# facebookresearch/nonrigid_nerf

Measured on NVIDIA H100. Metric: rays/sec (64c+128f samples, 8x256 MLP), example_sequence training step, higher is better.
Workload: dtype f16 (tensor-core operands; f32 accumulate)

## Files before the change

include/nrnerf_b200.h:

```cpp
#ifndef NRNERF_B200_H
#define NRNERF_B200_H

#include <stddef.h>
#include <stdint.h>

#ifdef __cplusplus
extern "C" {
#endif

#define NRN_ABI_VERSION 3

#define NRN_OK 0
#define NRN_E_INVALID (-1)
#define NRN_E_CUDA (-2)
#define NRN_E_DEVICE (-3)

int nrn_abi_version(void);
const char* nrn_last_error(void);

int nrn_device_error(int* code_out);

size_t nrn_packed_nerf_bytes(void);
size_t nrn_packed_bender_bytes(void);
int nrn_pack_nerf(const float* const* w, const float* const* b, int input_ch, int out_ch, void* packed,
                  void* stream);
int nrn_pack_bender(const float* const* net_w , const float* const* net_b ,
                    const float* const* rig_w , const float* const* rig_b , int latent_size,
                    void* packed, void* stream);

int nrn_get_rays(const float* c2w, const float* intrinsics, int height, int width, float* rays_o, float* rays_d, void* stream);
int nrn_pack_rays(const float* rays_o, const float* rays_d, float near, float far, int n_rays, float* rays, void* stream);
int nrn_ray_batch(const int64_t* pix, int n, const float* poses, const float* intrinsics, const int32_t* image_to_view,
                  const float* images, int height, int width, float* rays_o, float* rays_d, float* target, void* stream);
int nrn_median_visibility_index(const float* weights, int n_rays, int n_samples, int64_t* index, void* stream);

int nrn_sample_coarse(const float* rays, const float* t_rand, int n_rays, int n_samples, int lindisp,
                      float* z_vals, void* stream);

typedef struct NrnFieldArgs {
  const float* rays;
  const float* z_vals;
  const float* points;
  int64_t points_stride;
  const float* latents;
  int64_t latent_stride;
  int32_t n_rays;
  int32_t n_samples;
  const void* nerf_packed;
  const void* bender_packed;
  int32_t out_ch;
  int32_t use_cutoff;  float rigidity_cutoff;
  int32_t use_scaling; float scaling;
  int32_t use_removal; float removal_threshold;
  float* raw;
  float* initial_input_pts;
  float* input_pts;
  float* unmasked_offsets;
  float* masked_offsets;
  float* rigidity_mask;
  void* stash;
  void* stream;
  void* relu_mask;
} NrnFieldArgs;
int nrn_field_forward(const NrnFieldArgs* args);

typedef struct NrnCompositeArgs {
  const float* raw;
  const float* z_vals;
  const float* rays_d;
  int32_t rays_d_stride;
  const float* noise;
  int32_t n_rays, n_samples, channels, white_bkgd;
  float* rgb_map;
  float* disp_map;
  float* acc_map;
  float* depth_map;
  float* weights;
  float* alpha;
  int32_t n_importance;
  const float* u;
  float* z_vals_out;
  float* z_std;
  void* stream;
} NrnCompositeArgs;
int nrn_composite(const NrnCompositeArgs* args);

int nrn_sample_pdf(const float* bins, const float* weights, const float* u, int n, int nbins, int n_samples,
                   float* samples, void* stream);

typedef struct NrnCompositeBwdArgs {
  const float* raw; const float* z_vals; const float* rays_d; int32_t rays_d_stride; const float* noise;
  int32_t n_rays, n_samples, channels, white_bkgd;
  const float* d_rgb_map;
  const float* d_acc_map;
  float* d_raw;
  void* stream;
} NrnCompositeBwdArgs;
int nrn_composite_backward(const NrnCompositeBwdArgs* args);

size_t nrn_stash_bytes(int n_rays, int n_samples);
size_t nrn_grad_stash_bytes(int n_rays, int n_samples);
size_t nrn_relu_mask_bytes(int n_rays, int n_samples);
size_t nrn_wgrad_scratch_bytes(void);
int nrn_nerf_grad_floats(int out_ch);
int nrn_bender_grad_floats(void);
typedef struct NrnFieldBwdArgs {
  int32_t n_rays, n_samples, out_ch;
  const float* d_raw;
  const void* stash;
  void* grad_stash;
  float* wgrad_scratch;
  const void* nerf_packed;
  const void* bender_packed;
  const float* unmasked_offsets;
  const float* rigidity_mask;
  const float* d_unmasked_offsets;
  const float* d_rigidity_mask;
  int32_t use_cutoff;  float rigidity_cutoff;
  int32_t use_scaling; float scaling;
  float* nerf_grad;
  float* bender_grad;
  float* d_latents;
  void* stream;
  float* nerf_grad_head;
  int32_t accumulate_nerf, accumulate_bender;
  const void* relu_mask;
} NrnFieldBwdArgs;
int nrn_field_backward(const NrnFieldBwdArgs* args);

size_t nrn_div_stash_bytes(int n_rays, int n_samples);
size_t nrn_div_grad_stash_bytes(int n_rays, int n_samples);
typedef struct NrnDivArgs {
  int32_t n_rays, n_samples;
  const void* stash;
  const float* e;
  const float* unmasked_offsets;
  const float* rigidity_mask;
  const float* weights;
  int32_t weights_are_opacity_alpha;
  const float* const* net_w;
  const float* const* rig_w;
  void* tangent_stash;
  float* d; float* alpha; float* beta; float* tau_c;
  float* loss;
  const float* G;
  const float* g_ray;
  float* G_workspace;
  void* adjoint_stash;
  float* wgrad_scratch;
  float* d_unmasked_offsets;
  float* d_rigidity_mask;
  float* bender_grad;
  void* stream;
  int32_t accumulate_bender;
} NrnDivArgs;
int nrn_divergence_forward(const NrnDivArgs* args);
int nrn_divergence_backward(const NrnDivArgs* args);

typedef struct NrnRayLossArgs {
  int32_t n_rays, n_samples;
  const float* rgb;
  const float* rgb0;
  const float* target;
  const float* weights;
  const float* unmasked_offsets;
  const float* rigidity_mask;
  float lam_offsets;
  float lam_rigidity;
  float* loss;
  float* u_rgb; float* u_rgb0;
  float* u_unmasked_offsets;
  float* u_rigidity_mask;
  void* stream;
  const float* sched_step;
  float sched_n_iters;
  const float* divergence;
  float lam_divergence;
  float* u_divergence;
} NrnRayLossArgs;
int nrn_ray_loss(const NrnRayLossArgs* args);
int nrn_scale_rows(const float* g, const float* unit, float* out, int64_t n, int per_row, void* stream);
typedef struct NrnRayLossBwdArgs {
  int32_t n_rays, n_samples;
  const float* g;
  const float* u_rgb; const float* u_rgb0; const float* u_unmasked_offsets; const float* u_rigidity_mask; const float* u_divergence;
  float* d_rgb; float* d_rgb0; float* d_unmasked_offsets; float* d_rigidity_mask; float* d_divergence;
  void* stream;
} NrnRayLossBwdArgs;
int nrn_ray_loss_backward(const NrnRayLossBwdArgs* args);

typedef struct NrnAdamArgs {
  void* params;
  void* exp_avg;
  void* exp_avg_sq;
  const void* grad_ptrs;
  const void* blocks;
  int n_tensors, n_blocks;
  const void* lr;
  void* step;
  float beta1, beta2, eps;
  void* stream;
} NrnAdamArgs;
int nrn_adam_step(const NrnAdamArgs* args);

size_t nrn_peer_window_bytes(int64_t arena_floats, int64_t slot_floats);
int nrn_peer_alloc(size_t bytes, void** dev_ptr, void* ipc_handle_64bytes);
int nrn_peer_open(const void* ipc_handle_64bytes, void** dev_ptr);
int nrn_peer_close(void* dev_ptr);
int nrn_peer_free(void* dev_ptr);
typedef struct NrnPeerCtx {
  void* window[8];
  int32_t world, rank;
  int64_t arena_floats, slot_floats;
  void* state;
  float* reduced;
} NrnPeerCtx;
int nrn_peer_reduce_adam(const NrnPeerCtx* ctx, const NrnAdamArgs* adam);
int nrn_peer_gather_rows(const NrnPeerCtx* ctx, const float* local, int n_per_rank, float* out, void* stream);

int nrn_timing_enable(int on);
int nrn_timing_read(double* ms_sum, int* counts, int n_kinds);

#ifdef __cplusplus
}
#endif
#endif
```

nonrigid_nerf_b200/_lib.py:

```python
from __future__ import annotations

import ctypes as C
import os
import threading

_HERE = os.path.dirname(os.path.abspath(__file__))
LIB_PATH = os.path.join(_HERE, "libnrnerf_b200.so")
ABI_VERSION = 3

_f32p = C.POINTER(C.c_float)
_vp = C.c_void_p


class NrnFieldArgs(C.Structure):
    _fields_ = [
        ("rays", _vp), ("z_vals", _vp), ("points", _vp), ("points_stride", C.c_int64),
        ("latents", _vp), ("latent_stride", C.c_int64),
        ("n_rays", C.c_int32), ("n_samples", C.c_int32),
        ("nerf_packed", _vp), ("bender_packed", _vp),
        ("out_ch", C.c_int32),
        ("use_cutoff", C.c_int32), ("rigidity_cutoff", C.c_float),
        ("use_scaling", C.c_int32), ("scaling", C.c_float),
        ("use_removal", C.c_int32), ("removal_threshold", C.c_float),
        ("raw", _vp), ("initial_input_pts", _vp), ("input_pts", _vp), ("unmasked_offsets", _vp),
        ("masked_offsets", _vp), ("rigidity_mask", _vp),
        ("stash", _vp),
        ("stream", _vp),
        ("relu_mask", _vp),
    ]


class NrnFieldBwdArgs(C.Structure):
    _fields_ = [
        ("n_rays", C.c_int32), ("n_samples", C.c_int32), ("out_ch", C.c_int32),
        ("d_raw", _vp), ("stash", _vp), ("grad_stash", _vp), ("wgrad_scratch", _vp),
        ("nerf_packed", _vp), ("bender_packed", _vp),
        ("unmasked_offsets", _vp), ("rigidity_mask", _vp), ("d_unmasked_offsets", _vp), ("d_rigidity_mask", _vp),
        ("use_cutoff", C.c_int32), ("rigidity_cutoff", C.c_float),
        ("use_scaling", C.c_int32), ("scaling", C.c_float),
        ("nerf_grad", _vp), ("bender_grad", _vp), ("d_latents", _vp),
        ("stream", _vp),
        ("nerf_grad_head", _vp), ("accumulate_nerf", C.c_int32), ("accumulate_bender", C.c_int32),
        ("relu_mask", _vp),
    ]


class NrnDivArgs(C.Structure):
    _fields_ = [
        ("n_rays", C.c_int32), ("n_samples", C.c_int32),
        ("stash", _vp), ("e", _vp), ("unmasked_offsets", _vp), ("rigidity_mask", _vp), ("weights", _vp),
        ("weights_are_opacity_alpha", C.c_int32),
        ("net_w", C.POINTER(_vp)), ("rig_w", C.POINTER(_vp)),
        ("tangent_stash", _vp), ("d", _vp), ("alpha", _vp), ("beta", _vp), ("tau_c", _vp), ("loss", _vp),
        ("G", _vp), ("g_ray", _vp), ("G_workspace", _vp), ("adjoint_stash", _vp), ("wgrad_scratch", _vp), ("d_unmasked_offsets", _vp),
        ("d_rigidity_mask", _vp), ("bender_grad", _vp),
        ("stream", _vp),
        ("accumulate_bender", C.c_int32),
    ]


class NrnRayLossArgs(C.Structure):
    _fields_ = [
        ("n_rays", C.c_int32), ("n_samples", C.c_int32),
        ("rgb", _vp), ("rgb0", _vp), ("target", _vp), ("weights", _vp), ("unmasked_offsets", _vp), ("rigidity_mask", _vp),
        ("lam_offsets", C.c_float), ("lam_rigidity", C.c_float),
        ("loss", _vp), ("u_rgb", _vp), ("u_rgb0", _vp), ("u_unmasked_offsets", _vp), ("u_rigidity_mask", _vp),
        ("stream", _vp),
        ("sched_step", _vp), ("sched_n_iters", C.c_float), ("divergence", _vp), ("lam_divergence", C.c_float), ("u_divergence", _vp),
    ]


class NrnRayLossBwdArgs(C.Structure):
    _fields_ = [
        ("n_rays", C.c_int32), ("n_samples", C.c_int32), ("g", _vp),
        ("u_rgb", _vp), ("u_rgb0", _vp), ("u_unmasked_offsets", _vp), ("u_rigidity_mask", _vp), ("u_divergence", _vp),
        ("d_rgb", _vp), ("d_rgb0", _vp), ("d_unmasked_offsets", _vp), ("d_rigidity_mask", _vp), ("d_divergence", _vp),
        ("stream", _vp),
    ]


class NrnAdamArgs(C.Structure):
    _fields_ = [
        ("params", _vp), ("exp_avg", _vp), ("exp_avg_sq", _vp), ("grad_ptrs", _vp), ("blocks", _vp), ("n_tensors", C.c_int32), ("n_blocks", C.c_int32),
        ("lr", _vp), ("step", _vp), ("beta1", C.c_float), ("beta2", C.c_float), ("eps", C.c_float), ("stream", _vp),
    ]


class NrnPeerCtx(C.Structure):
    _fields_ = [
        ("window", _vp * 8), ("world", C.c_int32), ("rank", C.c_int32), ("arena_floats", C.c_int64), ("slot_floats", C.c_int64),
        ("state", _vp), ("reduced", _vp),
    ]


class NrnCompositeArgs(C.Structure):
    _fields_ = [
        ("raw", _vp), ("z_vals", _vp), ("rays_d", _vp), ("rays_d_stride", C.c_int32), ("noise", _vp),
        ("n_rays", C.c_int32), ("n_samples", C.c_int32), ("channels", C.c_int32), ("white_bkgd", C.c_int32),
        ("rgb_map", _vp), ("disp_map", _vp), ("acc_map", _vp), ("depth_map", _vp), ("weights", _vp), ("alpha", _vp),
        ("n_importance", C.c_int32), ("u", _vp), ("z_vals_out", _vp), ("z_std", _vp),
        ("stream", _vp),
    ]


class NrnCompositeBwdArgs(C.Structure):
    _fields_ = [
        ("raw", _vp), ("z_vals", _vp), ("rays_d", _vp), ("rays_d_stride", C.c_int32), ("noise", _vp),
        ("n_rays", C.c_int32), ("n_samples", C.c_int32), ("channels", C.c_int32), ("white_bkgd", C.c_int32),
        ("d_rgb_map", _vp), ("d_acc_map", _vp), ("d_raw", _vp),
        ("stream", _vp),
    ]


SYMBOLS = {
    "nrn_abi_version": (C.c_int, []),
    "nrn_last_error": (C.c_char_p, []),
    "nrn_device_error": (C.c_int, [C.POINTER(C.c_int)]),
    "nrn_packed_nerf_bytes": (C.c_size_t, []),
    "nrn_packed_bender_bytes": (C.c_size_t, []),
    "nrn_pack_nerf": (C.c_int, [C.POINTER(_vp), C.POINTER(_vp), C.c_int, C.c_int, _vp, _vp]),
    "nrn_pack_bender": (C.c_int, [C.POINTER(_vp), C.POINTER(_vp), C.POINTER(_vp), C.POINTER(_vp), C.c_int, _vp, _vp]),
    "nrn_sample_coarse": (C.c_int, [_vp, _vp, C.c_int, C.c_int, C.c_int, _vp, _vp]),
    "nrn_get_rays": (C.c_int, [_vp, _vp, C.c_int, C.c_int, _vp, _vp, _vp]),
    "nrn_pack_rays": (C.c_int, [_vp, _vp, C.c_float, C.c_float, C.c_int, _vp, _vp]),
    "nrn_ray_batch": (C.c_int, [_vp, C.c_int, _vp, _vp, _vp, _vp, C.c_int, C.c_int, _vp, _vp, _vp, _vp]),
    "nrn_median_visibility_index": (C.c_int, [_vp, C.c_int, C.c_int, _vp, _vp]),
    "nrn_field_forward": (C.c_int, [C.POINTER(NrnFieldArgs)]),
    "nrn_composite": (C.c_int, [C.POINTER(NrnCompositeArgs)]),
    "nrn_sample_pdf": (C.c_int, [_vp, _vp, _vp, C.c_int, C.c_int, C.c_int, _vp, _vp]),
    "nrn_composite_backward": (C.c_int, [C.POINTER(NrnCompositeBwdArgs)]),
    "nrn_stash_bytes": (C.c_size_t, [C.c_int, C.c_int]),
    "nrn_grad_stash_bytes": (C.c_size_t, [C.c_int, C.c_int]),
    "nrn_relu_mask_bytes": (C.c_size_t, [C.c_int, C.c_int]),
    "nrn_wgrad_scratch_bytes": (C.c_size_t, []),
    "nrn_nerf_grad_floats": (C.c_int, [C.c_int]),
    "nrn_bender_grad_floats": (C.c_int, []),
    "nrn_field_backward": (C.c_int, [C.POINTER(NrnFieldBwdArgs)]),
    "nrn_div_stash_bytes": (C.c_size_t, [C.c_int, C.c_int]),
    "nrn_div_grad_stash_bytes": (C.c_size_t, [C.c_int, C.c_int]),
    "nrn_divergence_forward": (C.c_int, [C.POINTER(NrnDivArgs)]),
    "nrn_divergence_backward": (C.c_int, [C.POINTER(NrnDivArgs)]),
    "nrn_ray_loss": (C.c_int, [C.POINTER(NrnRayLossArgs)]),
    "nrn_scale_rows": (C.c_int, [_vp, _vp, _vp, C.c_int64, C.c_int, _vp]),
    "nrn_ray_loss_backward": (C.c_int, [C.POINTER(NrnRayLossBwdArgs)]),
    "nrn_adam_step": (C.c_int, [C.POINTER(NrnAdamArgs)]),
    "nrn_peer_window_bytes": (C.c_size_t, [C.c_int64, C.c_int64]),
    "nrn_peer_alloc": (C.c_int, [C.c_size_t, C.POINTER(_vp), C.c_char_p]),
    "nrn_peer_open": (C.c_int, [C.c_char_p, C.POINTER(_vp)]),
    "nrn_peer_close": (C.c_int, [_vp]),
    "nrn_peer_free": (C.c_int, [_vp]),
    "nrn_peer_reduce_adam": (C.c_int, [C.POINTER(NrnPeerCtx), C.POINTER(NrnAdamArgs)]),
    "nrn_peer_gather_rows": (C.c_int, [C.POINTER(NrnPeerCtx), _vp, C.c_int, _vp, _vp]),
    "nrn_timing_enable": (C.c_int, [C.c_int]),
    "nrn_timing_read": (C.c_int, [C.POINTER(C.c_double), C.POINTER(C.c_int), C.c_int]),
}

KERNEL_KINDS = ("field_fwd", "field_dgrad", "wgrad", "composite", "composite_bwd", "divergence")


def timing_enable(on: bool) -> None:
    check(load().nrn_timing_enable(1 if on else 0), "timing_enable")


def timing_read():
    n = len(KERNEL_KINDS)
    ms = (C.c_double * n)()
    cnt = (C.c_int * n)()
    check(load().nrn_timing_read(ms, cnt, n), "timing_read")
    return {k: (ms[i], cnt[i]) for i, k in enumerate(KERNEL_KINDS)}

_lib = None
_lock = threading.Lock()


def load() -> C.CDLL:
    global _lib
    if _lib is not None:
        return _lib
    with _lock:
        if _lib is not None:
            return _lib
        if not os.path.exists(LIB_PATH):
            raise RuntimeError(
                f"nonrigid_nerf_b200: CUDA extension not found at {LIB_PATH}. There is no CPU/PyTorch fallback; "
                "build it with `make -C nonrigid_nerf_b200/csrc` (needs nvcc, sm_90a).")
        lib = C.CDLL(LIB_PATH)
        for name, (res, args) in SYMBOLS.items():
            fn = getattr(lib, name)
            fn.restype = res
            fn.argtypes = args
        v = lib.nrn_abi_version()
        if v != ABI_VERSION:
            raise RuntimeError(f"nonrigid_nerf_b200: ABI version mismatch (library {v}, bindings {ABI_VERSION})")
        _lib = lib
    return _lib


def check(rc: int, what: str = "") -> None:
    if rc != 0:
        msg = load().nrn_last_error()
        raise RuntimeError(f"nrnerf_b200 {what} failed (code {rc}): {msg.decode() if msg else '?'}")


def device_error_check() -> None:
    code = C.c_int(0)
    check(load().nrn_device_error(C.byref(code)), "device check")
```

nonrigid_nerf_b200/autograd.py:

```python
from __future__ import annotations

import ctypes as C
from typing import Dict, Optional, Tuple

import torch

from . import _lib, ops


def _knobs(net):
    bender = net.ray_bender[0]
    cutoff = getattr(bender, "rigidity_test_time_cutoff", None) if bender is not None else None
    scaling = getattr(bender, "test_time_scaling", None) if bender is not None else None
    removal = getattr(net, "test_time_nonrigid_object_removal_threshold", None)
    return cutoff, scaling, removal


def _flat_params(net, bender):
    ws, bs = ops.nerf_param_list(net)
    nerf = []
    for w, b in zip(ws, bs):
        nerf += [w, b]
    bend = []
    if bender is not None:
        net_w, net_b, rig_w, rig_b = ops.bender_param_list(bender)
        for i in range(4):
            bend += [net_w[i], net_b[i]]
        bend.append(net_w[4])
        for i in range(3):
            bend += [rig_w[i], rig_b[i]]
    return nerf, bend


def _split_flat(flat: torch.Tensor, like):
    out, o = [], 0
    for p in like:
        n = p.numel()
        out.append(flat[o:o + n].view_as(p))
        o += n
    assert o == flat.numel(), (o, flat.numel())
    return out


class _FieldTrainFn(torch.autograd.Function):

    @staticmethod
    def forward(ctx, net, rays, z_vals, latents, n_nerf, *params):
        bender = net.ray_bender[0]
        cutoff, scaling, removal = _knobs(net)
        if removal is not None:
            raise RuntimeError("nonrigid_nerf_b200: test_time_nonrigid_object_removal_threshold is a test-time knob; "
                               "it is not differentiable")
        nerf_pack = ops.pack_nerf(net)
        bender_pack = ops.pack_bender(bender) if bender is not None else None
        out_ch = net.output_linear.weight.shape[0]
        n, s = z_vals.shape
        lib = _lib.load()
        stash = torch.empty(lib.nrn_stash_bytes(n, s), dtype=torch.uint8, device=z_vals.device)
        relu_mask = torch.empty(lib.nrn_relu_mask_bytes(n, s), dtype=torch.uint8, device=z_vals.device)
        raw, det = ops.field_forward(rays, z_vals, latents, nerf_pack, bender_pack, out_ch, cutoff, scaling, None, True, stash,
                                     relu_mask)
        ctx.net, ctx.n_nerf = net, n_nerf
        ctx.shape = (n, s, out_ch)
        ctx.knobs = (cutoff, scaling)
        ctx.packs = (nerf_pack, bender_pack)
        ctx.stash = stash
        ctx.relu_mask = relu_mask
        ctx.params = params
        ctx.set_materialize_grads(False)
        if bender is not None:
            _register_stash(det["unmasked_offsets"], stash)
            ctx.save_for_backward(det["unmasked_offsets"], det["rigidity_mask"])
            outs = (raw, det["unmasked_offsets"], det["rigidity_mask"], det["initial_input_pts"], det["input_pts"],
                    det["masked_offsets"])
            ctx.mark_non_differentiable(*outs[3:])
        else:
            outs = (raw, det["initial_input_pts"], det["input_pts"])
            ctx.mark_non_differentiable(*outs[1:])
        return outs

    @staticmethod
    def backward(ctx, d_raw, *rest):
        net = ctx.net
        bender = net.ray_bender[0]
        n, s, out_ch = ctx.shape
        nerf_pack, bender_pack = ctx.packs
        cutoff, scaling = ctx.knobs
        dev = ctx.stash.device
        lib = _lib.load()
        d_un = d_rig = None
        if bender is not None:
            d_un, d_rig = rest[0], rest[1]
        if d_raw is None:
            d_raw = torch.zeros(n, s, out_ch, dtype=torch.float32, device=dev)
        a = _lib.NrnFieldBwdArgs()
        a.n_rays, a.n_samples, a.out_ch = n, s, out_ch
        d_raw = d_raw.contiguous().float()
        a.d_raw = d_raw.data_ptr()
        a.stash, a.relu_mask = ctx.stash.data_ptr(), ctx.relu_mask.data_ptr()
        gstash = torch.empty(lib.nrn_grad_stash_bytes(n, s), dtype=torch.uint8, device=dev)
        scratch = torch.empty(lib.nrn_wgrad_scratch_bytes(), dtype=torch.uint8, device=dev)
        a.grad_stash, a.wgrad_scratch = gstash.data_ptr(), scratch.data_ptr()
        a.nerf_packed = nerf_pack.data_ptr()
        nerf_p = list(ctx.params[:ctx.n_nerf])
        pts_dst = _arena_destination(nerf_p[:-2]) if all(p.requires_grad for p in nerf_p) else None
        head_dst = _arena_destination(nerf_p[-2:]) if pts_dst is not None else None
        nerf_grad = None
        if head_dst is not None:
            a.nerf_grad, a.nerf_grad_head, a.accumulate_nerf = pts_dst, head_dst, 1
        else:
            nerf_grad = torch.empty(lib.nrn_nerf_grad_floats(out_ch), dtype=torch.float32, device=dev)
            a.nerf_grad = nerf_grad.data_ptr()
        bend_grad = d_lat = None
        bend_in_place = False
        keep = [d_raw]
        if bender is not None:
            un, rig = ctx.saved_tensors
            a.bender_packed = bender_pack.data_ptr()
            a.unmasked_offsets, a.rigidity_mask = un.data_ptr(), rig.data_ptr()
            if d_un is not None:
                d_un = d_un.contiguous().float()
                a.d_unmasked_offsets = d_un.data_ptr()
                keep.append(d_un)
            if d_rig is not None:
                d_rig = d_rig.contiguous().float()
                a.d_rigidity_mask = d_rig.data_ptr()
                keep.append(d_rig)
            if cutoff is not None:
                a.use_cutoff, a.rigidity_cutoff = 1, float(cutoff)
            if scaling is not None:
                a.use_scaling, a.scaling = 1, float(scaling)
            bend_dst = _bender_arena(bender)
            if bend_dst is not None:
                a.bender_grad, a.accumulate_bender, bend_in_place = bend_dst, 1, True
            else:
                bend_grad = torch.empty(lib.nrn_bender_grad_floats(), dtype=torch.float32, device=dev)
                a.bender_grad = bend_grad.data_ptr()
            d_lat = torch.empty(n, ops.LATENT, dtype=torch.float32, device=dev)
            a.d_latents = d_lat.data_ptr()
        a.stream = torch.cuda.current_stream().cuda_stream
        with torch.cuda.device(dev):
            _lib.check(lib.nrn_field_backward(C.byref(a)), "field_backward")
        if nerf_grad is None:
            grads = [None] * len(nerf_p)
        else:
            grads = [g if p.requires_grad else None for g, p in zip(_split_flat(nerf_grad, nerf_p), nerf_p)]
        if bender is not None:
            bend_p = list(ctx.params[ctx.n_nerf:])
            if bend_in_place:
                grads += [None] * len(bend_p)
            else:
                grads += [g if p.requires_grad else None for g, p in zip(_split_flat(bend_grad, bend_p), bend_p)]
        return (None, None, None, d_lat, None, *grads)


def _arena_destination(params):
    from .optim import arena_destination
    return arena_destination(list(params))


def _bender_arena(bender):
    _, bend_p = _flat_params_bender(bender)
    if not all(p.requires_grad for p in bend_p):
        return None
    return _arena_destination(bend_p)


class _LatentGatherFn(torch.autograd.Function):

    @staticmethod
    def forward(ctx, timestep, *latents):
        z = latents[0].numel()
        base, contiguous = latents[0].data_ptr(), True
        for i, l in enumerate(latents):
            if l.data_ptr() != base + 4 * z * i or l.dtype != torch.float32 or not l.is_contiguous():
                contiguous = False
                break
        if contiguous and latents[0].untyped_storage().nbytes() >= latents[0].storage_offset() * 4 + 4 * z * len(latents):
            table = latents[0].detach().as_strided((len(latents), z), (z, 1))
        else:
            table = torch.stack([l.detach() for l in latents], 0)
        ctx.save_for_backward(timestep)
        ctx.latents = latents
        ctx.z = z
        return torch.index_select(table, 0, timestep)

    @staticmethod
    def backward(ctx, d_sel):
        (timestep,) = ctx.saved_tensors
        latents, z = ctx.latents, ctx.z
        t = len(latents)
        dst = _arena_destination(latents) if all(l.requires_grad for l in latents) else None
        if dst is not None:
            g0 = latents[0].grad
            g0.as_strided((t, z), (z, 1)).index_add_(0, timestep, d_sel.contiguous().float())
            return (None,) * (t + 1)
        g = torch.zeros(t, z, dtype=torch.float32, device=d_sel.device).index_add_(0, timestep, d_sel.float())
        return (None, *[g[i] if l.requires_grad else None for i, l in enumerate(latents)])


def gather_latents(latents, timestep: torch.Tensor) -> torch.Tensor:
    return _LatentGatherFn.apply(timestep, *latents)


_STASH_BY_PTR = {}


def _register_stash(unmasked: torch.Tensor, stash: torch.Tensor) -> None:
    import weakref
    for k in [k for k, v in _STASH_BY_PTR.items() if v() is None]:
        del _STASH_BY_PTR[k]
    _STASH_BY_PTR[unmasked.data_ptr()] = weakref.ref(stash)


def lookup_stash(unmasked: torch.Tensor) -> Optional[torch.Tensor]:
    fn = unmasked.grad_fn
    for _ in range(8):
        if fn is None:
            break
        stash = getattr(fn, "stash", None)
        if isinstance(stash, torch.Tensor):
            return stash
        nxt = [f for f, _ in fn.next_functions if f is not None]
        fn = nxt[0] if len(nxt) == 1 else None
    ref = _STASH_BY_PTR.get(unmasked.data_ptr())
    return ref() if ref is not None else None


class _DivergenceFn(torch.autograd.Function):

    @staticmethod
    def forward(ctx, unmasked, rigidity, weights, e, stash, bender, w_is_alpha, *bend_p):
        n, s = unmasked.shape[0], unmasked.shape[1]
        dev = unmasked.device
        lib = _lib.load()
        a = _lib.NrnDivArgs()
        a.n_rays, a.n_samples = n, s
        un = unmasked.detach().contiguous().float()
        rg = rigidity.detach().contiguous().float()
        w = weights.detach().contiguous().float()
        e = e.contiguous().float()
        net_w, _, rig_w, _ = ops.bender_param_list(bender)
        net_arr = ops._ptr_array([t.detach() for t in net_w])
        rig_arr = ops._ptr_array([t.detach() for t in rig_w])
        tan = torch.empty(lib.nrn_div_stash_bytes(n, s), dtype=torch.uint8, device=dev)
        scal = torch.empty(4, n * s, dtype=torch.float32, device=dev)
        loss = torch.empty(n, dtype=torch.float32, device=dev)
        a.stash, a.e, a.unmasked_offsets, a.rigidity_mask, a.weights = stash.data_ptr(), e.data_ptr(), un.data_ptr(), rg.data_ptr(), w.data_ptr()
        a.weights_are_opacity_alpha = 1 if w_is_alpha else 0
        a.net_w, a.rig_w = net_arr, rig_arr
        a.tangent_stash = tan.data_ptr()
        a.d, a.alpha, a.beta, a.tau_c = (scal[i].data_ptr() for i in range(4))
        a.loss = loss.data_ptr()
        a.stream = torch.cuda.current_stream().cuda_stream
        with torch.cuda.device(dev):
            _lib.check(lib.nrn_divergence_forward(C.byref(a)), "divergence_forward")
        ctx.keep = (un, rg, w, e, stash, tan, scal, bender)
        ctx.bend_p = bend_p
        ctx.w_is_alpha = bool(w_is_alpha)
        ctx.shape = (n, s)
        ctx.in_shapes = (unmasked.shape, rigidity.shape)
        return loss

    @staticmethod
    def backward(ctx, g):
        un, rg, w, e, stash, tan, scal, bender = ctx.keep
        n, s = ctx.shape
        dev = un.device
        lib = _lib.load()
        g = g.reshape(n).contiguous().float()
        G = torch.empty(n * s, dtype=torch.float32, device=dev)
        a = _lib.NrnDivArgs()
        a.n_rays, a.n_samples = n, s
        net_w, _, rig_w, _ = ops.bender_param_list(bender)
        net_arr = ops._ptr_array([t.detach() for t in net_w])
        rig_arr = ops._ptr_array([t.detach() for t in rig_w])
        a.stash, a.e, a.unmasked_offsets, a.rigidity_mask, a.weights = stash.data_ptr(), e.data_ptr(), un.data_ptr(), rg.data_ptr(), w.data_ptr()
        a.weights_are_opacity_alpha = 1 if ctx.w_is_alpha else 0
        a.net_w, a.rig_w = net_arr, rig_arr
        a.tangent_stash = tan.data_ptr()
        a.d, a.alpha, a.beta, a.tau_c = (scal[i].data_ptr() for i in range(4))
        a.g_ray, a.G_workspace = g.data_ptr(), G.data_ptr()
        adj = torch.empty(lib.nrn_div_grad_stash_bytes(n, s), dtype=torch.uint8, device=dev)
        scratch = torch.empty(lib.nrn_wgrad_scratch_bytes(), dtype=torch.uint8, device=dev)
        d_un = torch.empty(n * s, 3, dtype=torch.float32, device=dev)
        d_rg = torch.empty(n * s, dtype=torch.float32, device=dev)
        bend_dst = _bender_arena(bender)
        bend_grad = None
        if bend_dst is not None:
            a.bender_grad, a.accumulate_bender = bend_dst, 1
        else:
            bend_grad = torch.empty(lib.nrn_bender_grad_floats(), dtype=torch.float32, device=dev)
            a.bender_grad = bend_grad.data_ptr()
        a.adjoint_stash, a.wgrad_scratch = adj.data_ptr(), scratch.data_ptr()
        a.d_unmasked_offsets, a.d_rigidity_mask = d_un.data_ptr(), d_rg.data_ptr()
        a.stream = torch.cuda.current_stream().cuda_stream
        with torch.cuda.device(dev):
            _lib.check(lib.nrn_divergence_backward(C.byref(a)), "divergence_backward")
        bend_p = list(ctx.bend_p)
        if bend_grad is None:
            pgrads = [None] * len(bend_p)
        else:
            pgrads = [g if p.requires_grad else None for g, p in zip(_split_flat(bend_grad, bend_p), bend_p)]
        return (d_un.view(ctx.in_shapes[0]), d_rg.view(ctx.in_shapes[1]), None, None, None, None, None, *pgrads)


def divergence_loss(unmasked: torch.Tensor, rigidity: torch.Tensor, weights: Optional[torch.Tensor], bender,
                    e: Optional[torch.Tensor] = None, opacity_alpha: Optional[torch.Tensor] = None) -> torch.Tensor:
    stash = lookup_stash(unmasked)
    if stash is None:
        raise RuntimeError("nonrigid_nerf_b200: no activation stash for these offsets -- the fused divergence term needs the "
                           "un-chunked coarse pass of the current differentiable render() call (N_rand <= chunk)")
    n, s = unmasked.shape[0], unmasked.shape[1]
    if e is None:
        e = torch.randn(n * s, 3, device=unmasked.device)
    _, bend_p = _flat_params_bender(bender)
    if opacity_alpha is not None:
        return _DivergenceFn.apply(unmasked, rigidity, opacity_alpha, e, stash, bender, True, *bend_p)
    return _DivergenceFn.apply(unmasked, rigidity, weights, e, stash, bender, False, *bend_p)


def _flat_params_bender(bender):
    net_w, net_b, rig_w, rig_b = ops.bender_param_list(bender)
    bend = []
    for i in range(4):
        bend += [net_w[i], net_b[i]]
    bend.append(net_w[4])
    for i in range(3):
        bend += [rig_w[i], rig_b[i]]
    return None, bend


class _RayLossFn(torch.autograd.Function):

    @staticmethod
    def forward(ctx, rgb, rgb0, target, weights, unmasked, rigidity, lam_o, lam_r, sched_step, sched_n_iters, div, lam_div):
        n = rgb.shape[0]
        dev = rgb.device
        lib = _lib.load()
        a = _lib.NrnRayLossArgs()
        keep = [rgb.detach().contiguous().float(), target.contiguous().float()]
        a.rgb, a.target = keep[0].data_ptr(), keep[1].data_ptr()
        u_rgb = torch.empty(n, 3, dtype=torch.float32, device=dev)
        a.u_rgb = u_rgb.data_ptr()
        u_rgb0 = u_off = u_rig = u_div = None
        if rgb0 is not None:
            keep.append(rgb0.detach().contiguous().float())
            a.rgb0 = keep[-1].data_ptr()
            u_rgb0 = torch.empty(n, 3, dtype=torch.float32, device=dev)
            a.u_rgb0 = u_rgb0.data_ptr()
        s = 1
        if unmasked is not None:
            s = unmasked.shape[1]
            keep += [weights.detach().contiguous().float(), unmasked.detach().contiguous().float(), rigidity.detach().contiguous().float()]
            a.weights, a.unmasked_offsets, a.rigidity_mask = (t.data_ptr() for t in keep[-3:])
            u_off = torch.empty(n, s, 3, dtype=torch.float32, device=dev)
            u_rig = torch.empty(rigidity.shape, dtype=torch.float32, device=dev)
            a.u_unmasked_offsets, a.u_rigidity_mask = u_off.data_ptr(), u_rig.data_ptr()
        a.n_rays, a.n_samples = n, s
        a.lam_offsets, a.lam_rigidity = float(lam_o), float(lam_r)
        if sched_step is not None:
            keep.append(sched_step.detach().float().contiguous())
            a.sched_step, a.sched_n_iters = keep[-1].data_ptr(), float(sched_n_iters)
        if div is not None:
            keep.append(div.detach().contiguous().float())
            u_div = torch.empty(n, dtype=torch.float32, device=dev)
            a.divergence, a.lam_divergence, a.u_divergence = keep[-1].data_ptr(), float(lam_div), u_div.data_ptr()
        loss = torch.empty(n, dtype=torch.float32, device=dev)
        a.loss = loss.data_ptr()
        a.stream = torch.cuda.current_stream().cuda_stream
        with torch.cuda.device(dev):
            _lib.check(lib.nrn_ray_loss(C.byref(a)), "ray_loss")
        ctx.units = (u_rgb, u_rgb0, u_off, u_rig, u_div)
        ctx.ns = (n, s)
        return loss

    @staticmethod
    def backward(ctx, g):
        lib = _lib.load()
        g = g.contiguous().float()
        a = _lib.NrnRayLossBwdArgs()
        a.n_rays, a.n_samples = ctx.ns
        a.g = g.data_ptr()
        outs = [None if u is None else torch.empty_like(u) for u in ctx.units]
        names = ("rgb", "rgb0", "unmasked_offsets", "rigidity_mask", "divergence")
        for nm, u, o in zip(names, ctx.units, outs):
            if u is not None:
                setattr(a, "u_" + nm, u.data_ptr())
                setattr(a, "d_" + nm, o.data_ptr())
        a.stream = torch.cuda.current_stream().cuda_stream
        with torch.cuda.device(g.device):
            _lib.check(lib.nrn_ray_loss_backward(C.byref(a)), "ray_loss_backward")
        d_rgb, d_rgb0, d_off, d_rig, d_div = outs
        return d_rgb, d_rgb0, None, None, d_off, d_rig, None, None, None, None, d_div, None


def ray_loss(rgb, rgb0, target, weights=None, unmasked=None, rigidity=None, lam_offsets=0.0, lam_rigidity=0.0,
             sched_step: Optional[torch.Tensor] = None, sched_n_iters: float = 1.0, divergence: Optional[torch.Tensor] = None,
             lam_divergence: float = 0.0):
    return _RayLossFn.apply(rgb, rgb0, target, weights, unmasked, rigidity, lam_offsets, lam_rigidity, sched_step, sched_n_iters,
                            divergence, lam_divergence)


class _CompositeFn(torch.autograd.Function):
    @staticmethod
    def forward(ctx, raw, z_vals, rays_d, noise, white_bkgd, n_importance, u):
        o = ops.composite(raw, z_vals, rays_d, noise, white_bkgd, n_importance, u, True)
        ctx.save_for_backward(raw, z_vals, rays_d, noise if noise is not None else raw.new_empty(0))
        ctx.has_noise = noise is not None
        ctx.white = bool(white_bkgd)
        ctx.set_materialize_grads(False)
        outs = [o["rgb_map"], o["acc_map"], o["disp_map"], o["depth_map"], o["weights"], o["alpha"]]
        if n_importance > 0:
            outs += [o["z_vals_out"], o["z_std"]]
        ctx.mark_non_differentiable(*outs[2:])
        return tuple(outs)

    @staticmethod
    def backward(ctx, d_rgb, d_acc, *unsupported):
        raw, z_vals, rays_d, noise = ctx.saved_tensors
        if d_rgb is None and d_acc is None:
            return None, None, None, None, None, None, None
        if d_rgb is None:
            d_rgb = torch.zeros(raw.shape[0], 3, dtype=torch.float32, device=raw.device)
        d_raw = ops.composite_backward(raw, z_vals, rays_d, noise if ctx.has_noise else None, ctx.white, d_rgb, d_acc)
        return d_raw, None, None, None, None, None, None


def _needs_grad(net, latents) -> bool:
    if not torch.is_grad_enabled():
        return False
    bender = net.ray_bender[0]
    if latents is not None and latents.requires_grad:
        return True
    if any(p.requires_grad for p in net.parameters()):
        return True
    return bender is not None and any(p.requires_grad for p in bender.parameters())


def field(net, rays: torch.Tensor, z_vals: torch.Tensor, latents: Optional[torch.Tensor],
          want_details: bool) -> Tuple[torch.Tensor, Dict[str, torch.Tensor]]:
    bender = net.ray_bender[0]
    if not _needs_grad(net, latents):
        return field_rays(net, rays, z_vals, latents, want_details)
    nerf_p, bend_p = _flat_params(net, bender)
    outs = _FieldTrainFn.apply(net, rays, z_vals, latents, len(nerf_p), *nerf_p, *bend_p)
    if bender is not None:
        raw, un, rig, init, bent, masked = outs
        details = {"initial_input_pts": init, "unmasked_offsets": un, "rigidity_mask": rig, "masked_offsets": masked,
                   "input_pts": bent}
    else:
        raw, init, bent = outs
        details = {"initial_input_pts": init, "input_pts": bent}
    return raw, (details if want_details else {})


def field_rays(net, rays, z_vals, latents, want_details):
    bender = net.ray_bender[0]
    cutoff, scaling, removal = _knobs(net)
    nerf_pack = ops.pack_nerf(net)
    bender_pack = ops.pack_bender(bender) if bender is not None else None
    out_ch = net.output_linear.weight.shape[0]
    return ops.field_forward(rays, z_vals, latents, nerf_pack, bender_pack, out_ch, cutoff, scaling, removal, want_details)


def field_points(net, pts, latents, want_details):
    if _needs_grad(net, latents):
        raise RuntimeError("nonrigid_nerf_b200: the point-wise NeRF.forward / run_network entry is inference-only; "
                           "differentiable rendering goes through render() / render_rays()")
    bender = net.ray_bender[0]
    cutoff, scaling, removal = _knobs(net)
    nerf_pack = ops.pack_nerf(net)
    bender_pack = ops.pack_bender(bender) if bender is not None else None
    out_ch = net.output_linear.weight.shape[0]
    return ops.field_forward_points(pts, latents, nerf_pack, bender_pack, out_ch, cutoff, scaling, removal, want_details)


def composite(raw, z_vals, rays_d, noise=None, white_bkgd=False, n_importance=0, u=None) -> Dict[str, torch.Tensor]:
    if torch.is_grad_enabled() and raw.requires_grad:
        outs = _CompositeFn.apply(raw, z_vals, rays_d, noise, white_bkgd, n_importance, u)
        keys = ["rgb_map", "acc_map", "disp_map", "depth_map", "weights", "alpha"] + (["z_vals_out", "z_std"] if n_importance > 0 else [])
        return dict(zip(keys, outs))
    return ops.composite(raw, z_vals, rays_d, noise, white_bkgd, n_importance, u, True)
```

nonrigid_nerf_b200/csrc/c_abi.cu:

```cuda
#include <cstdarg>
#include <cstdio>
#include <cstring>
#include <cstdlib>
#include "../../include/nrnerf_b200.h"
#include "nrn_common.cuh"
#include "pack.cuh"
#include "ray_ops.cuh"
#include "wgrad.cuh"
#include "div.cuh"
#include "loss.cuh"
#include "adam.cuh"
#include "peer.cuh"

namespace nrn {
cudaError_t launch_field_fwd(const FieldFwdParams& p, bool has_bender, int num_sms, cudaStream_t stream);
cudaError_t launch_field_bwd(const FieldBwdParams& p, bool has_bender, int num_sms, cudaStream_t stream);
}

namespace {

thread_local char g_err[512] = "";

int fail(int code, const char* fmt, ...) {
  va_list ap;
  va_start(ap, fmt);
  vsnprintf(g_err, sizeof(g_err), fmt, ap);
  va_end(ap);
  return code;
}
int cuda_fail(cudaError_t e, const char* what) {
  return fail(NRN_E_CUDA, "%s: %s", what, cudaGetErrorString(e));
}

constexpr int kMaxDevices = 64;
struct DeviceState {
  int* err_word = nullptr;
  int num_sms = 0;
};
DeviceState g_dev[kMaxDevices];

int device_state(DeviceState** out) {
  int dev = 0;
  cudaError_t e = cudaGetDevice(&dev);
  if (e != cudaSuccess) return cuda_fail(e, "cudaGetDevice");
  if (dev < 0 || dev >= kMaxDevices) return fail(NRN_E_INVALID, "device index %d out of range", dev);
  DeviceState& s = g_dev[dev];
  if (!s.err_word) {
    cudaDeviceProp prop;
    e = cudaGetDeviceProperties(&prop, dev);
    if (e != cudaSuccess) return cuda_fail(e, "cudaGetDeviceProperties");
    if (prop.major != 9 || prop.minor != 0)
      return fail(NRN_E_INVALID, "nrnerf_b200 is built for sm_90a (H100) only, found sm_%d%d", prop.major, prop.minor);
    s.num_sms = prop.multiProcessorCount;
    if (const char* g = getenv("NRN_GRID")) { const int v = atoi(g); if (v > 0 && v < s.num_sms) s.num_sms = v; }
    e = cudaMalloc(&s.err_word, 4 * sizeof(int));
    if (e != cudaSuccess) return cuda_fail(e, "cudaMalloc(err word)");
    e = cudaMemset(s.err_word, 0, 4 * sizeof(int));
    if (e != cudaSuccess) return cuda_fail(e, "cudaMemset(err word)");
  }
  *out = &s;
  return NRN_OK;
}

bool aligned16(const void* p) { return (reinterpret_cast<uintptr_t>(p) & 15u) == 0; }

struct TimedLaunch {
  cudaEvent_t a, b;
  int kind;
};
bool g_timing = false;
TimedLaunch g_timed[4096];
int g_timed_n = 0;
struct ScopedTimer {
  int idx = -1;
  cudaStream_t st;
  ScopedTimer(int kind, cudaStream_t s) : st(s) {
    if (!g_timing || g_timed_n >= 4096) return;
    TimedLaunch& t = g_timed[g_timed_n];
    if (cudaEventCreate(&t.a) != cudaSuccess || cudaEventCreate(&t.b) != cudaSuccess) return;
    t.kind = kind;
    idx = g_timed_n++;
    record(t.a);
  }
  ~ScopedTimer() {
    if (idx >= 0) record(g_timed[idx].b);
  }
  void record(cudaEvent_t ev) {
    cudaStreamCaptureStatus cs = cudaStreamCaptureStatusNone;
    cudaStreamIsCapturing(st, &cs);
    cudaEventRecordWithFlags(ev, st, cs == cudaStreamCaptureStatusActive ? cudaEventRecordExternal : cudaEventRecordDefault);
  }
};

}

extern "C" {

int nrn_abi_version(void) { return NRN_ABI_VERSION; }
const char* nrn_last_error(void) { return g_err; }

int nrn_device_error(int* code_out) {
  DeviceState* ds;
  int rc = device_state(&ds);
  if (rc) return rc;
  cudaError_t e = cudaDeviceSynchronize();
  if (e != cudaSuccess) return cuda_fail(e, "cudaDeviceSynchronize");
  int code = 0;
  e = cudaMemcpy(&code, ds->err_word, sizeof(int), cudaMemcpyDeviceToHost);
  if (e != cudaSuccess) return cuda_fail(e, "cudaMemcpy(err word)");
  if (code) cudaMemset(ds->err_word, 0, sizeof(int));
  if (code_out) *code_out = code;
  if (code) return fail(NRN_E_DEVICE, "device-side protocol error: wait id %d timed out", code);
  return NRN_OK;
}

size_t nrn_packed_nerf_bytes(void) { return nrn::kNerfPackedBytes; }
size_t nrn_packed_bender_bytes(void) { return nrn::kBendPackedBytes; }

int nrn_pack_nerf(const float* const* w, const float* const* b, int input_ch, int out_ch, void* packed, void* stream) {
  if (!w || !b || !packed) return fail(NRN_E_INVALID, "nrn_pack_nerf: null argument");
  if (input_ch < 1 || input_ch > 63) return fail(NRN_E_INVALID, "nrn_pack_nerf: input_ch=%d unsupported (1..63; multires=10 gives 63)", input_ch);
  if (out_ch < 4 || out_ch > 16) return fail(NRN_E_INVALID, "nrn_pack_nerf: out_ch=%d unsupported", out_ch);
  if (!aligned16(packed)) return fail(NRN_E_INVALID, "nrn_pack_nerf: packed buffer must be 16-byte aligned");
  nrn::NerfSrc src;
  for (int i = 0; i < 9; ++i) {
    if (!w[i] || !b[i]) return fail(NRN_E_INVALID, "nrn_pack_nerf: null layer %d", i);
    src.w[i] = w[i];
    src.b[i] = b[i];
  }
  cudaError_t e = nrn::launch_pack_nerf(src, input_ch, out_ch, packed, static_cast<cudaStream_t>(stream));
  return e == cudaSuccess ? NRN_OK : cuda_fail(e, "pack_nerf_kernel");
}

int nrn_pack_bender(const float* const* net_w, const float* const* net_b, const float* const* rig_w,
                    const float* const* rig_b, int latent_size, void* packed, void* stream) {
  if (!net_w || !net_b || !rig_w || !rig_b || !packed) return fail(NRN_E_INVALID, "nrn_pack_bender: null argument");
  if (latent_size != nrn::kLatent) return fail(NRN_E_INVALID, "nrn_pack_bender: ray_bending_latent_size=%d unsupported (32)", latent_size);
  if (!aligned16(packed)) return fail(NRN_E_INVALID, "nrn_pack_bender: packed buffer must be 16-byte aligned");
  nrn::BenderSrc src;
  for (int i = 0; i < 5; ++i) src.net_w[i] = net_w[i];
  for (int i = 0; i < 4; ++i) src.net_b[i] = net_b[i];
  for (int i = 0; i < 3; ++i) { src.rig_w[i] = rig_w[i]; src.rig_b[i] = rig_b[i]; }
  cudaError_t e = nrn::launch_pack_bender(src, packed, static_cast<cudaStream_t>(stream));
  return e == cudaSuccess ? NRN_OK : cuda_fail(e, "pack_bender_kernel");
}

int nrn_sample_coarse(const float* rays, const float* t_rand, int n_rays, int n_samples, int lindisp, float* z_vals,
                      void* stream) {
  if (n_rays < 0 || n_samples < 1) return fail(NRN_E_INVALID, "nrn_sample_coarse: bad sizes n=%d S=%d", n_rays, n_samples);
  if (n_rays == 0) return NRN_OK;
  if (!rays || !z_vals) return fail(NRN_E_INVALID, "nrn_sample_coarse: null argument");
  cudaError_t e = nrn::launch_sample_coarse(rays, t_rand, n_rays, n_samples, lindisp, z_vals, static_cast<cudaStream_t>(stream));
  return e == cudaSuccess ? NRN_OK : cuda_fail(e, "sample_coarse_kernel");
}

int nrn_get_rays(const float* c2w, const float* K, int H, int W, float* rays_o, float* rays_d, void* stream) {
  if (H < 0 || W < 0) return fail(NRN_E_INVALID, "nrn_get_rays: bad sizes");
  if (H == 0 || W == 0) return NRN_OK;
  if (!c2w || !K || !rays_o || !rays_d) return fail(NRN_E_INVALID, "nrn_get_rays: null argument");
  const cudaError_t e = nrn::launch_get_rays(c2w, K, H, W, rays_o, rays_d, static_cast<cudaStream_t>(stream));
  return e == cudaSuccess ? NRN_OK : cuda_fail(e, "get_rays_kernel");
}

int nrn_pack_rays(const float* rays_o, const float* rays_d, float near, float far, int n_rays, float* rays, void* stream) {
  if (n_rays < 0) return fail(NRN_E_INVALID, "nrn_pack_rays: bad size");
  if (n_rays == 0) return NRN_OK;
  if (!rays_o || !rays_d || !rays) return fail(NRN_E_INVALID, "nrn_pack_rays: null argument");
  const cudaError_t e = nrn::launch_pack_rays(rays_o, rays_d, near, far, n_rays, rays, static_cast<cudaStream_t>(stream));
  return e == cudaSuccess ? NRN_OK : cuda_fail(e, "pack_rays_kernel");
}

int nrn_ray_batch(const int64_t* pix, int n, const float* poses, const float* K, const int32_t* image_to_view, const float* images,
                  int H, int W, float* rays_o, float* rays_d, float* target, void* stream) {
  if (n < 0 || H < 1 || W < 1) return fail(NRN_E_INVALID, "nrn_ray_batch: bad sizes");
  if (n == 0) return NRN_OK;
  if (!pix || !poses || !K || !rays_o || !rays_d || (images && !target)) return fail(NRN_E_INVALID, "nrn_ray_batch: null argument");
  static_assert(sizeof(long long) == sizeof(int64_t), "int64");
  const cudaError_t e = nrn::launch_ray_batch(reinterpret_cast<const long long*>(pix), n, poses, K, image_to_view, images, H, W, rays_o, rays_d,
                                              target, static_cast<cudaStream_t>(stream));
  return e == cudaSuccess ? NRN_OK : cuda_fail(e, "ray_batch_kernel");
}

int nrn_median_visibility_index(const float* weights, int n_rays, int n_samples, int64_t* index, void* stream) {
  if (n_rays < 0 || n_samples < 1) return fail(NRN_E_INVALID, "nrn_median_visibility_index: bad sizes");
  if (n_rays == 0) return NRN_OK;
  if (!weights || !index) return fail(NRN_E_INVALID, "nrn_median_visibility_index: null argument");
  const cudaError_t e = nrn::launch_median_index(weights, n_rays, n_samples, reinterpret_cast<long long*>(index), static_cast<cudaStream_t>(stream));
  return e == cudaSuccess ? NRN_OK : cuda_fail(e, "median_index_kernel");
}

int nrn_field_forward(const NrnFieldArgs* a) {
  if (!a) return fail(NRN_E_INVALID, "nrn_field_forward: null args");
  if (a->n_rays < 0 || a->n_samples < 1) return fail(NRN_E_INVALID, "nrn_field_forward: bad sizes n=%d S=%d", a->n_rays, a->n_samples);
  if (a->n_rays == 0) return NRN_OK;
  if (!a->nerf_packed || !a->raw) return fail(NRN_E_INVALID, "nrn_field_forward: null argument");
  if (a->points) {
    if (a->n_samples != 1 || a->points_stride < 3) return fail(NRN_E_INVALID, "nrn_field_forward: point mode needs n_samples=1, stride>=3");
  } else if (!a->rays || !a->z_vals) {
    return fail(NRN_E_INVALID, "nrn_field_forward: null rays / z_vals");
  }
  if (a->bender_packed && !a->latents) return fail(NRN_E_INVALID, "nrn_field_forward: bender given without latents");
  if (a->out_ch < 4 || a->out_ch > 5) return fail(NRN_E_INVALID, "nrn_field_forward: out_ch=%d unsupported (4 or 5)", a->out_ch);
  if (!aligned16(a->nerf_packed) || (a->bender_packed && !aligned16(a->bender_packed)))
    return fail(NRN_E_INVALID, "nrn_field_forward: packed weights must be 16-byte aligned");
  if ((a->stash != nullptr) != (a->relu_mask != nullptr))
    return fail(NRN_E_INVALID, "nrn_field_forward: training needs both the stash and the ReLU mask buffer (relu_mask)");
  DeviceState* ds;
  int rc = device_state(&ds);
  if (rc) return rc;
  nrn::FieldFwdParams p{};
  p.rays = a->rays; p.z_vals = a->z_vals; p.pts = a->points; p.pts_stride = a->points_stride; p.latents = a->latents; p.latent_stride = a->latent_stride;
  p.n_rays = a->n_rays; p.S = a->n_samples;
  p.P = static_cast<long long>(a->n_rays) * a->n_samples;
  const long long tiles = (p.P + nrn::kTileM - 1) / nrn::kTileM;
  if (tiles > 0x7fffffffLL) return fail(NRN_E_INVALID, "nrn_field_forward: too many points");
  p.n_tiles = static_cast<int>(tiles);
  const uint8_t* np = static_cast<const uint8_t*>(a->nerf_packed);
  p.nerf_w = np; p.nerf_bias = reinterpret_cast<const float*>(np + nrn::kNerfWBytes);
  if (a->bender_packed) {
    const uint8_t* bp = static_cast<const uint8_t*>(a->bender_packed);
    p.bend_w = bp; p.bend_bias = reinterpret_cast<const float*>(bp + nrn::kBendWBytes);
  }
  p.cutoff = a->rigidity_cutoff; p.use_cutoff = a->use_cutoff;
  p.scaling = a->scaling; p.use_scaling = a->use_scaling;
  p.removal = a->removal_threshold; p.use_removal = a->use_removal;
  p.out_ch = a->out_ch;
  p.raw = a->raw; p.d_init = a->initial_input_pts; p.d_bent = a->input_pts; p.d_unmasked = a->unmasked_offsets;
  p.d_masked = a->masked_offsets; p.d_rigid = a->rigidity_mask;
  p.stash = static_cast<uint8_t*>(a->stash);
  p.relu_mask = static_cast<uint8_t*>(a->relu_mask);
  if (a->stash && a->points) return fail(NRN_E_INVALID, "nrn_field_forward: the training stash needs ray mode");
  p.err = ds->err_word;
  cudaError_t e;
  {
    ScopedTimer tm(0, static_cast<cudaStream_t>(a->stream));
    e = nrn::launch_field_fwd(p, a->bender_packed != nullptr, ds->num_sms, static_cast<cudaStream_t>(a->stream));
  }
  return e == cudaSuccess ? NRN_OK : cuda_fail(e, "field_fwd_kernel");
}

int nrn_composite(const NrnCompositeArgs* a) {
  if (!a) return fail(NRN_E_INVALID, "nrn_composite: null args");
  if (a->n_rays < 0 || a->n_samples < 1 || a->channels < 4) return fail(NRN_E_INVALID, "nrn_composite: bad sizes");
  if (a->n_rays == 0) return NRN_OK;
  if (!a->raw || !a->z_vals || !a->rays_d || !a->rgb_map || !a->disp_map || !a->acc_map) return fail(NRN_E_INVALID, "nrn_composite: null argument");
  if (a->n_importance < 0) return fail(NRN_E_INVALID, "nrn_composite: n_importance < 0");
  if (a->n_importance > 0 && (!a->z_vals_out || a->n_samples < 3)) return fail(NRN_E_INVALID, "nrn_composite: resampling needs z_vals_out and >= 3 samples");
  if (4 * a->n_samples + a->n_importance > 12000) return fail(NRN_E_INVALID, "nrn_composite: too many samples per ray");
  nrn::CompositeParams p{};
  p.raw = a->raw; p.z = a->z_vals; p.rays_d = a->rays_d; p.rays_d_stride = a->rays_d_stride; p.noise = a->noise;
  p.n = a->n_rays; p.S = a->n_samples; p.C = a->channels; p.white_bkgd = a->white_bkgd;
  p.rgb = a->rgb_map; p.disp = a->disp_map; p.acc = a->acc_map; p.depth = a->depth_map; p.weights = a->weights; p.alpha = a->alpha;
  p.n_imp = a->n_importance; p.u = a->u; p.z_out = a->z_vals_out; p.z_std = a->z_std;
  cudaError_t e; { ScopedTimer tm(3, static_cast<cudaStream_t>(a->stream)); e = nrn::launch_composite(p, static_cast<cudaStream_t>(a->stream)); }
  return e == cudaSuccess ? NRN_OK : cuda_fail(e, "composite_kernel");
}

int nrn_sample_pdf(const float* bins, const float* weights, const float* u, int n, int nbins, int n_samples, float* samples,
                   void* stream) {
  if (n < 0 || nbins < 2 || n_samples < 1 || nbins > 4000) return fail(NRN_E_INVALID, "nrn_sample_pdf: bad sizes");
  if (n == 0) return NRN_OK;
  if (!bins || !weights || !samples) return fail(NRN_E_INVALID, "nrn_sample_pdf: null argument");
  cudaError_t e = nrn::launch_sample_pdf(bins, weights, u, n, nbins, n_samples, samples, static_cast<cudaStream_t>(stream));
  return e == cudaSuccess ? NRN_OK : cuda_fail(e, "sample_pdf_kernel");
}

int nrn_composite_backward(const NrnCompositeBwdArgs* a) {
  if (!a) return fail(NRN_E_INVALID, "nrn_composite_backward: null args");
  if (a->n_rays < 0 || a->n_samples < 1 || a->channels < 4 || a->n_samples > 12000) return fail(NRN_E_INVALID, "nrn_composite_backward: bad sizes");
  if (a->n_rays == 0) return NRN_OK;
  if (!a->raw || !a->z_vals || !a->rays_d || !a->d_rgb_map || !a->d_raw) return fail(NRN_E_INVALID, "nrn_composite_backward: null argument");
  nrn::CompositeBwdParams p{};
  p.raw = a->raw; p.z = a->z_vals; p.rays_d = a->rays_d; p.rays_d_stride = a->rays_d_stride; p.noise = a->noise;
  p.n = a->n_rays; p.S = a->n_samples; p.C = a->channels; p.white_bkgd = a->white_bkgd;
  p.d_rgb = a->d_rgb_map; p.d_acc = a->d_acc_map; p.d_raw = a->d_raw;
  cudaError_t e; { ScopedTimer tm(4, static_cast<cudaStream_t>(a->stream)); e = nrn::launch_composite_bwd(p, static_cast<cudaStream_t>(a->stream)); }
  return e == cudaSuccess ? NRN_OK : cuda_fail(e, "composite_bwd_kernel");
}

static long long even_tiles(int n_rays, int n_samples) {
  const long long P = static_cast<long long>(n_rays) * n_samples;
  const long long tiles = (P + nrn::kTileM - 1) / nrn::kTileM;
  return (tiles + 1) & ~1LL;
}
size_t nrn_stash_bytes(int n_rays, int n_samples) { return static_cast<size_t>(even_tiles(n_rays, n_samples)) * nrn::kStashTileBytes; }
size_t nrn_grad_stash_bytes(int n_rays, int n_samples) { return static_cast<size_t>(even_tiles(n_rays, n_samples)) * nrn::kGradTileBytes; }
size_t nrn_relu_mask_bytes(int n_rays, int n_samples) { return static_cast<size_t>(even_tiles(n_rays, n_samples)) * nrn::kMaskTileBytes; }
size_t nrn_wgrad_scratch_bytes(void) { return static_cast<size_t>(nrn::kWgMaxCtas) * nrn::kWgScratchFloats * sizeof(float); }
int nrn_nerf_grad_floats(int out_ch) { return 256 * 63 + 256 + 6 * (65536 + 256) + 256 * 319 + 256 + out_ch * 257; }
int nrn_bender_grad_floats(void) { return 16193; }

int nrn_field_backward(const NrnFieldBwdArgs* a) {
  if (!a) return fail(NRN_E_INVALID, "nrn_field_backward: null args");
  if (a->n_rays < 0 || a->n_samples < 1) return fail(NRN_E_INVALID, "nrn_field_backward: bad sizes");
  if (a->out_ch < 4 || a->out_ch > 5) return fail(NRN_E_INVALID, "nrn_field_backward: out_ch=%d unsupported", a->out_ch);
  if (!a->nerf_packed || !a->nerf_grad) return fail(NRN_E_INVALID, "nrn_field_backward: null argument");
  const bool bend = a->bender_packed != nullptr;
  if (bend && (!a->unmasked_offsets || !a->rigidity_mask || !a->bender_grad || !a->d_latents))
    return fail(NRN_E_INVALID, "nrn_field_backward: bender needs unmasked_offsets, rigidity_mask, bender_grad, d_latents");
  if (a->n_rays > 0 && !a->relu_mask) return fail(NRN_E_INVALID, "nrn_field_backward: null relu_mask (the ReLU masks of the forward call)");
  DeviceState* ds;
  int rc = device_state(&ds);
  if (rc) return rc;
  if (ds->num_sms + 16 > nrn::kWgMaxCtas) return fail(NRN_E_INVALID, "nrn_field_backward: %d SMs exceed the scratch layout", ds->num_sms);
  cudaStream_t st = static_cast<cudaStream_t>(a->stream);
  const int nerf_n = nrn_nerf_grad_floats(a->out_ch);
  const int bend_n = bend ? nrn_bender_grad_floats() : 0;
  cudaError_t e;
  if (bend) {
    e = cudaMemsetAsync(a->d_latents, 0, sizeof(float) * static_cast<size_t>(a->n_rays) * nrn::kLatent, st);
    if (e != cudaSuccess) return cuda_fail(e, "memset d_latents");
  }
  if (a->n_rays == 0) {
    e = cudaSuccess;
    if (!a->accumulate_nerf) {
      const int head_n = a->nerf_grad_head ? a->out_ch * 257 : 0;
      e = cudaMemsetAsync(a->nerf_grad, 0, sizeof(float) * (nerf_n - head_n), st);
      if (e == cudaSuccess && head_n) e = cudaMemsetAsync(a->nerf_grad_head, 0, sizeof(float) * head_n, st);
    }
    if (e == cudaSuccess && bend && !a->accumulate_bender) e = cudaMemsetAsync(a->bender_grad, 0, sizeof(float) * bend_n, st);
    return e == cudaSuccess ? NRN_OK : cuda_fail(e, "memset grads");
  }
  if (!a->d_raw || !a->stash || !a->grad_stash || !a->wgrad_scratch) return fail(NRN_E_INVALID, "nrn_field_backward: null argument");
  float* amax = reinterpret_cast<float*>(ds->err_word + 1);
  nrn::FieldBwdParams p{};
  p.P = static_cast<long long>(a->n_rays) * a->n_samples;
  p.n_tiles = static_cast<int>((p.P + nrn::kTileM - 1) / nrn::kTileM);
  p.S = a->n_samples; p.n_rays = a->n_rays; p.out_ch = a->out_ch;
  p.d_raw = a->d_raw; p.amax = amax;
  p.stash = static_cast<const uint8_t*>(a->stash); p.gstash = static_cast<uint8_t*>(a->grad_stash);
  p.nerf_wT = static_cast<const uint8_t*>(a->nerf_packed) + nrn::kNerfTOffset;
  if (bend) p.bend_wT = static_cast<const uint8_t*>(a->bender_packed) + nrn::kBendTOffset;
  p.unmasked = a->unmasked_offsets; p.rigidity = a->rigidity_mask;
  p.d_unmasked_up = a->d_unmasked_offsets; p.d_rigid_up = a->d_rigidity_mask;
  p.cutoff = a->rigidity_cutoff; p.use_cutoff = a->use_cutoff; p.scaling = a->scaling; p.use_scaling = a->use_scaling;
  p.d_latents = a->d_latents; p.err = ds->err_word;
  p.relu_mask = static_cast<const uint8_t*>(a->relu_mask);
  e = nrn::launch_absmax(a->d_raw, p.P * a->out_ch, amax, st);
  if (e == cudaSuccess && bend && p.d_unmasked_up) e = nrn::launch_absmax(p.d_unmasked_up, p.P * 3, amax, st, true);
  if (e == cudaSuccess && bend && p.d_rigid_up) e = nrn::launch_absmax(p.d_rigid_up, p.P, amax, st, true);
  if (e != cudaSuccess) return cuda_fail(e, "absmax_kernel");
  { ScopedTimer tm(1, st); e = nrn::launch_field_bwd(p, bend, ds->num_sms, st); }
  if (e != cudaSuccess) return cuda_fail(e, "field_bwd_kernel");
  nrn::WgradParams w{};
  w.stash = p.stash; w.gstash = p.gstash; w.scratch = a->wgrad_scratch; w.amax = amax; w.n_tiles = p.n_tiles; w.err = ds->err_word;
  const nrn::WgradDst dst{a->nerf_grad, a->nerf_grad_head, a->bender_grad, nerf_n, bend_n, a->accumulate_nerf, a->accumulate_bender};
  { ScopedTimer tm(2, st); e = nrn::launch_wgrad(w, bend, ds->num_sms, dst, a->out_ch, st); }
  return e == cudaSuccess ? NRN_OK : cuda_fail(e, "wgrad_kernel");
}

static long long point_tiles(int n_rays, int n_samples) {
  return (static_cast<long long>(n_rays) * n_samples + nrn::kTileM - 1) / nrn::kTileM;
}
size_t nrn_div_stash_bytes(int n_rays, int n_samples) { return static_cast<size_t>(point_tiles(n_rays, n_samples)) * nrn::kTanTileBytes; }
size_t nrn_div_grad_stash_bytes(int n_rays, int n_samples) { return static_cast<size_t>(point_tiles(n_rays, n_samples)) * nrn::kAdjTileBytes; }

static int fill_div(const NrnDivArgs* a, nrn::DivParams& p, const char* who) {
  if (!a) return fail(NRN_E_INVALID, "%s: null args", who);
  if (a->n_rays < 0 || a->n_samples < 1) return fail(NRN_E_INVALID, "%s: bad sizes", who);
  if (!a->stash || !a->e || !a->unmasked_offsets || !a->rigidity_mask || !a->weights || !a->net_w || !a->rig_w || !a->tangent_stash ||
      !a->d || !a->alpha || !a->beta || !a->tau_c)
    return fail(NRN_E_INVALID, "%s: null argument", who);
  p.P = static_cast<long long>(a->n_rays) * a->n_samples;
  p.S = a->n_samples; p.n_rays = a->n_rays;
  p.stash = static_cast<const uint8_t*>(a->stash);
  p.e = a->e; p.unmasked = a->unmasked_offsets; p.rigidity = a->rigidity_mask; p.w = a->weights; p.w_is_alpha = a->weights_are_opacity_alpha != 0;
  for (int i = 0; i < 5; ++i) { if (!a->net_w[i]) return fail(NRN_E_INVALID, "%s: null weight", who); p.net_w[i] = a->net_w[i]; }
  for (int i = 0; i < 3; ++i) { if (!a->rig_w[i]) return fail(NRN_E_INVALID, "%s: null weight", who); p.rig_w[i] = a->rig_w[i]; }
  p.tan = static_cast<uint8_t*>(a->tangent_stash);
  p.d = a->d; p.adot = a->alpha; p.beta = a->beta; p.tauc = a->tau_c;
  return NRN_OK;
}

int nrn_divergence_forward(const NrnDivArgs* a) {
  nrn::DivParams p{};
  int rc = fill_div(a, p, "nrn_divergence_forward");
  if (rc) return rc;
  if (!a->loss) return fail(NRN_E_INVALID, "nrn_divergence_forward: null loss");
  cudaStream_t st = static_cast<cudaStream_t>(a->stream);
  cudaError_t e = cudaMemsetAsync(a->loss, 0, sizeof(float) * static_cast<size_t>(a->n_rays), st);
  if (e != cudaSuccess) return cuda_fail(e, "memset loss");
  p.loss = a->loss;
  { ScopedTimer tm(5, st); e = nrn::launch_div_fwd(p, st); }
  return e == cudaSuccess ? NRN_OK : cuda_fail(e, "div_fwd_kernel");
}

int nrn_divergence_backward(const NrnDivArgs* a) {
  nrn::DivParams p{};
  int rc = fill_div(a, p, "nrn_divergence_backward");
  if (rc) return rc;
  if ((!a->G && !(a->g_ray && a->G_workspace)) || !a->adjoint_stash || !a->wgrad_scratch || !a->d_unmasked_offsets || !a->d_rigidity_mask ||
      !a->bender_grad)
    return fail(NRN_E_INVALID, "nrn_divergence_backward: null argument");
  DeviceState* ds;
  rc = device_state(&ds);
  if (rc) return rc;
  cudaStream_t st = static_cast<cudaStream_t>(a->stream);
  float* amax = reinterpret_cast<float*>(ds->err_word + 2);
  p.G = a->G ? a->G : a->G_workspace; p.amax = amax; p.adj = static_cast<uint8_t*>(a->adjoint_stash);
  p.d_unmasked = a->d_unmasked_offsets; p.d_rigid = a->d_rigidity_mask;
  cudaError_t e = a->G ? nrn::launch_absmax(a->G, p.P, amax, st) : nrn::launch_div_G(p, a->g_ray, a->G_workspace, amax, st);
  if (e != cudaSuccess) return cuda_fail(e, "absmax_kernel");
  { ScopedTimer tm(5, st); e = nrn::launch_div_bwd(p, st); }
  if (e != cudaSuccess) return cuda_fail(e, "div_bwd_kernel");
  nrn::WgradParams w{};
  w.stash = p.tan; w.gstash = p.adj; w.scratch = a->wgrad_scratch; w.amax = amax; w.compact = 1;
  w.n_tiles = static_cast<int>((p.P + nrn::kTileM - 1) / nrn::kTileM); w.err = ds->err_word;
  const nrn::WgradDst dst{nullptr, nullptr, a->bender_grad, 0, nrn_bender_grad_floats(), 0, a->accumulate_bender};
  { ScopedTimer tm(2, st); e = nrn::launch_wgrad(w, true, ds->num_sms, dst, 5, st); }
  return e == cudaSuccess ? NRN_OK : cuda_fail(e, "wgrad_kernel (divergence)");
}

int nrn_ray_loss(const NrnRayLossArgs* a) {
  if (!a) return fail(NRN_E_INVALID, "nrn_ray_loss: null args");
  if (a->n_rays < 0 || a->n_samples < 1) return fail(NRN_E_INVALID, "nrn_ray_loss: bad sizes");
  if (a->n_rays == 0) return NRN_OK;
  if (!a->rgb || !a->target || !a->loss || !a->u_rgb || (a->rgb0 && !a->u_rgb0)) return fail(NRN_E_INVALID, "nrn_ray_loss: null argument");
  if (a->unmasked_offsets && (!a->weights || !a->rigidity_mask || !a->u_unmasked_offsets || !a->u_rigidity_mask))
    return fail(NRN_E_INVALID, "nrn_ray_loss: the offsets term needs weights, rigidity_mask and both gradient outputs");
  if (a->divergence && !a->u_divergence) return fail(NRN_E_INVALID, "nrn_ray_loss: the divergence term needs u_divergence");
  if (a->sched_step && !(a->sched_n_iters > 0.f)) return fail(NRN_E_INVALID, "nrn_ray_loss: sched_n_iters must be positive");
  nrn::RayLossParams p{};
  p.n = a->n_rays; p.S = a->n_samples;
  p.rgb = a->rgb; p.rgb0 = a->rgb0; p.target = a->target; p.w = a->weights; p.off = a->unmasked_offsets; p.rig = a->rigidity_mask;
  p.lam_o = a->lam_offsets; p.lam_r = a->lam_rigidity;
  p.sched_step = a->sched_step; p.sched_n_iters = a->sched_n_iters; p.div = a->divergence; p.lam_div = a->lam_divergence; p.u_div = a->u_divergence;
  p.loss = a->loss; p.u_rgb = a->u_rgb; p.u_rgb0 = a->u_rgb0; p.u_off = a->u_unmasked_offsets; p.u_rig = a->u_rigidity_mask;
  cudaError_t e = nrn::launch_ray_loss(p, static_cast<cudaStream_t>(a->stream));
  return e == cudaSuccess ? NRN_OK : cuda_fail(e, "ray_loss_kernel");
}

int nrn_ray_loss_backward(const NrnRayLossBwdArgs* a) {
  if (!a) return fail(NRN_E_INVALID, "nrn_ray_loss_backward: null args");
  if (a->n_rays < 0 || a->n_samples < 1) return fail(NRN_E_INVALID, "nrn_ray_loss_backward: bad sizes");
  if (a->n_rays == 0) return NRN_OK;
  if (!a->g) return fail(NRN_E_INVALID, "nrn_ray_loss_backward: null upstream gradient");
  nrn::RayLossBwdParams p{};
  p.n = a->n_rays; p.S = a->n_samples; p.g = a->g;
  const float* u[5] = {a->u_rgb, a->u_rgb0, a->u_unmasked_offsets, a->u_rigidity_mask, a->u_divergence};
  float* d[5] = {a->d_rgb, a->d_rgb0, a->d_unmasked_offsets, a->d_rigidity_mask, a->d_divergence};
  for (int k = 0; k < 5; ++k) {
    if ((u[k] == nullptr) != (d[k] == nullptr)) return fail(NRN_E_INVALID, "nrn_ray_loss_backward: unit / output pair %d half given", k);
    p.u[k] = u[k]; p.d[k] = d[k];
  }
  const cudaError_t e = nrn::launch_ray_loss_bwd(p, static_cast<cudaStream_t>(a->stream));
  return e == cudaSuccess ? NRN_OK : cuda_fail(e, "ray_loss_bwd_kernel");
}

int nrn_scale_rows(const float* g, const float* unit, float* out, int64_t n, int per_row, void* stream) {
  if (n < 0 || per_row < 1) return fail(NRN_E_INVALID, "nrn_scale_rows: bad sizes");
  if (n == 0) return NRN_OK;
  if (!g || !unit || !out) return fail(NRN_E_INVALID, "nrn_scale_rows: null argument");
  cudaError_t e = nrn::launch_ray_loss_scale(g, unit, out, n, per_row, static_cast<cudaStream_t>(stream));
  return e == cudaSuccess ? NRN_OK : cuda_fail(e, "ray_loss_scale_kernel");
}

static int fill_adam(const NrnAdamArgs* a, nrn::AdamParams& p, const char* who, bool need_grads);
int nrn_adam_step(const NrnAdamArgs* a) {
  nrn::AdamParams p{};
  const int rc = fill_adam(a, p, "nrn_adam_step", true);
  if (rc) return rc;
  const cudaError_t e = nrn::launch_adam(p, a->n_tensors, a->n_blocks, static_cast<cudaStream_t>(a->stream));
  return e == cudaSuccess ? NRN_OK : cuda_fail(e, "adam_kernel");
}

static int fill_adam(const NrnAdamArgs* a, nrn::AdamParams& p, const char* who, bool need_grads) {
  if (!a) return fail(NRN_E_INVALID, "%s: null args", who);
  if (a->n_blocks < 0 || a->n_tensors < 0) return fail(NRN_E_INVALID, "%s: n_tensors = %d, n_blocks = %d", who, a->n_tensors, a->n_blocks);
  if (!a->params || !a->exp_avg || !a->exp_avg_sq || (need_grads && !a->grad_ptrs) || !a->blocks || !a->lr || !a->step)
    return fail(NRN_E_INVALID, "%s: null buffer", who);
  if (!(a->beta1 >= 0.f && a->beta1 < 1.f && a->beta2 >= 0.f && a->beta2 < 1.f && a->eps >= 0.f))
    return fail(NRN_E_INVALID, "%s: betas / eps out of range", who);
  p.params = static_cast<float*>(a->params); p.exp_avg = static_cast<float*>(a->exp_avg); p.exp_avg_sq = static_cast<float*>(a->exp_avg_sq);
  p.grads = static_cast<const float* const*>(a->grad_ptrs); p.blocks = static_cast<const nrn::AdamBlock*>(a->blocks);
  p.lr = static_cast<const float*>(a->lr); p.step = static_cast<long long*>(a->step);
  p.beta1 = a->beta1; p.beta2 = a->beta2; p.eps = a->eps;
  return NRN_OK;
}

size_t nrn_peer_window_bytes(int64_t arena_floats, int64_t slot_floats) {
  if (arena_floats < 0 || slot_floats < 0) return 0;
  const size_t slot_bytes = (static_cast<size_t>(slot_floats) * 4 + 255) / 256 * 256;
  return nrn::kPeerFlagBytes + 2 * slot_bytes + (static_cast<size_t>(arena_floats) * 4 + 255) / 256 * 256;
}

int nrn_peer_alloc(size_t bytes, void** dev_ptr, void* ipc_handle) {
  if (!dev_ptr || !ipc_handle || bytes < nrn::kPeerFlagBytes) return fail(NRN_E_INVALID, "nrn_peer_alloc: bad arguments");
  static_assert(sizeof(cudaIpcMemHandle_t) == 64, "CUDA IPC handle size");
  void* p = nullptr;
  cudaError_t e = cudaMalloc(&p, bytes);
  if (e != cudaSuccess) return cuda_fail(e, "cudaMalloc(peer window)");
  e = cudaMemset(p, 0, bytes);
  if (e == cudaSuccess) e = cudaDeviceSynchronize();
  cudaIpcMemHandle_t h;
  if (e == cudaSuccess) e = cudaIpcGetMemHandle(&h, p);
  if (e != cudaSuccess) { cudaFree(p); return cuda_fail(e, "cudaIpcGetMemHandle"); }
  memcpy(ipc_handle, &h, sizeof(h));
  *dev_ptr = p;
  return NRN_OK;
}

int nrn_peer_open(const void* ipc_handle, void** dev_ptr) {
  if (!ipc_handle || !dev_ptr) return fail(NRN_E_INVALID, "nrn_peer_open: null argument");
  cudaIpcMemHandle_t h;
  memcpy(&h, ipc_handle, sizeof(h));
  void* p = nullptr;
  const cudaError_t e = cudaIpcOpenMemHandle(&p, h, cudaIpcMemLazyEnablePeerAccess);
  if (e != cudaSuccess) return cuda_fail(e, "cudaIpcOpenMemHandle (peer-to-peer access between the GPUs of this node is required)");
  *dev_ptr = p;
  return NRN_OK;
}

int nrn_peer_close(void* dev_ptr) {
  if (!dev_ptr) return NRN_OK;
  const cudaError_t e = cudaIpcCloseMemHandle(dev_ptr);
  return e == cudaSuccess ? NRN_OK : cuda_fail(e, "cudaIpcCloseMemHandle");
}

int nrn_peer_free(void* dev_ptr) {
  if (!dev_ptr) return NRN_OK;
  const cudaError_t e = cudaFree(dev_ptr);
  return e == cudaSuccess ? NRN_OK : cuda_fail(e, "cudaFree(peer window)");
}

static int fill_peer(const NrnPeerCtx* c, nrn::PeerCtx& p, const char* who) {
  if (!c) return fail(NRN_E_INVALID, "%s: null context", who);
  if (c->world < 1 || c->world > nrn::kPeerMaxRanks || c->rank < 0 || c->rank >= c->world)
    return fail(NRN_E_INVALID, "%s: world = %d, rank = %d (at most %d ranks of one node)", who, c->world, c->rank, nrn::kPeerMaxRanks);
  if (!c->state || c->arena_floats < 0 || c->slot_floats < 0) return fail(NRN_E_INVALID, "%s: bad context", who);
  for (int r = 0; r < c->world; ++r) {
    if (!c->window[r]) return fail(NRN_E_INVALID, "%s: window of rank %d not mapped", who, r);
    p.window[r] = static_cast<uint8_t*>(c->window[r]);
  }
  p.world = c->world; p.rank = c->rank;
  p.slot_off = nrn::kPeerFlagBytes;
  p.slot_bytes = (static_cast<size_t>(c->slot_floats) * 4 + 255) / 256 * 256;
  p.arena_off = p.slot_off + 2 * p.slot_bytes;
  return NRN_OK;
}

int nrn_peer_reduce_adam(const NrnPeerCtx* c, const NrnAdamArgs* a) {
  nrn::PeerCtx pc{};
  int rc = fill_peer(c, pc, "nrn_peer_reduce_adam");
  if (rc) return rc;
  nrn::AdamParams p{};
  rc = fill_adam(a, p, "nrn_peer_reduce_adam", false);
  if (rc) return rc;
  if (!c->reduced) return fail(NRN_E_INVALID, "nrn_peer_reduce_adam: null workspace");
  DeviceState* ds;
  rc = device_state(&ds);
  if (rc) return rc;
  uint32_t* state = static_cast<uint32_t*>(c->state);
  const cudaError_t e = nrn::launch_peer_reduce_adam(pc, p, a->n_tensors, a->n_blocks, c->arena_floats, state, c->reduced, state + 3,
                                                     ds->err_word, static_cast<cudaStream_t>(a->stream));
  return e == cudaSuccess ? NRN_OK : cuda_fail(e, "peer_adam_kernel");
}

int nrn_peer_gather_rows(const NrnPeerCtx* c, const float* local, int n_per_rank, float* out, void* stream) {
  nrn::PeerCtx pc{};
  int rc = fill_peer(c, pc, "nrn_peer_gather_rows");
  if (rc) return rc;
  if (n_per_rank < 0 || n_per_rank > c->slot_floats) return fail(NRN_E_INVALID, "nrn_peer_gather_rows: %d floats per rank exceed the slot (%lld)", n_per_rank, (long long)c->slot_floats);
  if (n_per_rank == 0) return NRN_OK;
  if (!local || !out) return fail(NRN_E_INVALID, "nrn_peer_gather_rows: null argument");
  DeviceState* ds;
  rc = device_state(&ds);
  if (rc) return rc;
  const cudaError_t e = nrn::launch_peer_gather(pc, static_cast<uint32_t*>(c->state), local, n_per_rank, out, ds->err_word, static_cast<cudaStream_t>(stream));
  return e == cudaSuccess ? NRN_OK : cuda_fail(e, "peer_collect_kernel");
}

int nrn_timing_enable(int on) {
  if (on) {
    for (int i = 0; i < g_timed_n; ++i) { cudaEventDestroy(g_timed[i].a); cudaEventDestroy(g_timed[i].b); }
    g_timed_n = 0;
  }
  g_timing = on != 0;
  return NRN_OK;
}

int nrn_timing_read(double* ms_sum, int* counts, int n_kinds) {
  if (!ms_sum || !counts || n_kinds < 1) return fail(NRN_E_INVALID, "nrn_timing_read: bad arguments");
  for (int k = 0; k < n_kinds; ++k) { ms_sum[k] = 0.0; counts[k] = 0; }
  for (int i = 0; i < g_timed_n; ++i) {
    cudaError_t e = cudaEventSynchronize(g_timed[i].b);
    if (e != cudaSuccess) return cuda_fail(e, "cudaEventSynchronize");
    float ms = 0.f;
    e = cudaEventElapsedTime(&ms, g_timed[i].a, g_timed[i].b);
    if (e != cudaSuccess) return cuda_fail(e, "cudaEventElapsedTime");
    if (g_timed[i].kind < n_kinds) { ms_sum[g_timed[i].kind] += ms; counts[g_timed[i].kind] += 1; }
  }
  return NRN_OK;
}

}
```

nonrigid_nerf_b200/csrc/div.cu:

```cuda
#include <cuda_fp16.h>
#include "nrn_common.cuh"
#include "div.cuh"

namespace nrn {

namespace {

constexpr int kDivThreads = 128;
constexpr int kW0x = 0;
constexpr int kW1 = kW0x + 64 * 4;
constexpr int kW2 = kW1 + 4096;
constexpr int kW3 = kW2 + 4096;
constexpr int kW4 = kW3 + 4096;
constexpr int kR0 = kW4 + 192;
constexpr int kR1 = kR0 + 128;
constexpr int kR2 = kR1 + 1024;
constexpr int kWTotal = kR2 + 32;
constexpr int kActFloats = 64 * kDivThreads;

constexpr int kTE = 0, kT1 = 6 * kChunkBytes, kT2 = 18 * kChunkBytes, kT3 = 30 * kChunkBytes, kT4 = 38 * kChunkBytes;
constexpr int kA4 = 0, kA3 = 2 * kChunkBytes, kA2 = 10 * kChunkBytes, kA1 = 20 * kChunkBytes, kA0 = 32 * kChunkBytes;

__device__ __forceinline__ void load_weights(float* sw, const DivParams& p) {
  for (int i = threadIdx.x; i < 64 * 4; i += blockDim.x) sw[kW0x + i] = (i & 3) < 3 ? p.net_w[0][(i >> 2) * 35 + (i & 3)] : 0.f;
  for (int i = threadIdx.x; i < 4096; i += blockDim.x) {
    sw[kW1 + i] = p.net_w[1][i];
    sw[kW2 + i] = p.net_w[2][i];
    sw[kW3 + i] = p.net_w[3][i];
  }
  for (int i = threadIdx.x; i < 192; i += blockDim.x) sw[kW4 + i] = p.net_w[4][i];
  for (int i = threadIdx.x; i < 32 * 4; i += blockDim.x) sw[kR0 + i] = (i & 3) < 3 ? p.rig_w[0][(i >> 2) * 3 + (i & 3)] : 0.f;
  for (int i = threadIdx.x; i < 1024; i += blockDim.x) sw[kR1 + i] = p.rig_w[1][i];
  for (int i = threadIdx.x; i < 32; i += blockDim.x) sw[kR2 + i] = p.rig_w[2][i];
}

__device__ __forceinline__ unsigned long long read_mask(const uint8_t* row, int nchunks) {
  unsigned long long m = 0ull;
  for (int c = 0; c < nchunks; ++c) {
    const uint4 w = __ldg(reinterpret_cast<const uint4*>(row + c * kChunkBytes));
    const uint32_t ww[4] = {w.x, w.y, w.z, w.w};
#pragma unroll
    for (int q = 0; q < 4; ++q) {
      if (ww[q] & 0x7fffu) m |= 1ull << (c * 8 + 2 * q);
      if (ww[q] & 0x7fff0000u) m |= 1ull << (c * 8 + 2 * q + 1);
    }
  }
  return m;
}

__device__ __forceinline__ uint32_t pk(float a, float b) {
  __half2 h = __floats2half2_rn(fminf(fmaxf(a, -65504.f), 65504.f), fminf(fmaxf(b, -65504.f), 65504.f));
  return *reinterpret_cast<uint32_t*>(&h);
}

template <int IN>
__device__ __forceinline__ void matvec(const float* W, const float (&in)[IN], float* act, int OUT) {
#pragma unroll 1
  for (int j0 = 0; j0 < OUT; j0 += 4) {
    float a0 = 0.f, a1 = 0.f, a2 = 0.f, a3 = 0.f;
#pragma unroll
    for (int k = 0; k < IN; k += 4) {
      const float4 w0 = *reinterpret_cast<const float4*>(W + (j0 + 0) * IN + k);
      const float4 w1 = *reinterpret_cast<const float4*>(W + (j0 + 1) * IN + k);
      const float4 w2 = *reinterpret_cast<const float4*>(W + (j0 + 2) * IN + k);
      const float4 w3 = *reinterpret_cast<const float4*>(W + (j0 + 3) * IN + k);
      a0 += w0.x * in[k] + w0.y * in[k + 1] + w0.z * in[k + 2] + w0.w * in[k + 3];
      a1 += w1.x * in[k] + w1.y * in[k + 1] + w1.z * in[k + 2] + w1.w * in[k + 3];
      a2 += w2.x * in[k] + w2.y * in[k + 1] + w2.z * in[k + 2] + w2.w * in[k + 3];
      a3 += w3.x * in[k] + w3.y * in[k + 1] + w3.z * in[k + 2] + w3.w * in[k + 3];
    }
    act[(j0 + 0) * kDivThreads] = a0; act[(j0 + 1) * kDivThreads] = a1;
    act[(j0 + 2) * kDivThreads] = a2; act[(j0 + 3) * kDivThreads] = a3;
  }
}
template <int NJ>
__device__ __forceinline__ void matvec_t(const float* W, const float (&in)[NJ], float* act, int NK) {
#pragma unroll 1
  for (int k0 = 0; k0 < NK; k0 += 4) {
    float a0 = 0.f, a1 = 0.f, a2 = 0.f, a3 = 0.f;
#pragma unroll
    for (int j = 0; j < NJ; ++j) {
      const float4 w = *reinterpret_cast<const float4*>(W + j * NK + k0);
      a0 += w.x * in[j]; a1 += w.y * in[j]; a2 += w.z * in[j]; a3 += w.w * in[j];
    }
    act[(k0 + 0) * kDivThreads] = a0; act[(k0 + 1) * kDivThreads] = a1;
    act[(k0 + 2) * kDivThreads] = a2; act[(k0 + 3) * kDivThreads] = a3;
  }
}
template <int N>
__device__ __forceinline__ void take(const float* act, unsigned long long mask, float scale, float (&out)[N], uint8_t* img_row) {
#pragma unroll
  for (int j = 0; j < N; ++j) out[j] = ((mask >> j) & 1ull) ? act[j * kDivThreads] * scale : 0.f;
#pragma unroll
  for (int c = 0; c < N / 8; ++c) {
    const uint4 v = make_uint4(pk(out[c * 8], out[c * 8 + 1]), pk(out[c * 8 + 2], out[c * 8 + 3]), pk(out[c * 8 + 4], out[c * 8 + 5]),
                               pk(out[c * 8 + 6], out[c * 8 + 7]));
    *reinterpret_cast<uint4*>(img_row + c * kChunkBytes) = v;
  }
}

}

__global__ void __launch_bounds__(kDivThreads) div_fwd_kernel(const DivParams p) {
  extern __shared__ __align__(16) float sm[];
  float* sw = sm;
  float* act = sm + kWTotal + threadIdx.x;
  load_weights(sw, p);
  __syncthreads();
  const long long tile = blockIdx.x;
  const int row = threadIdx.x;
  const long long pt = tile * kTileM + row;
  const bool valid = pt < p.P;
  const uint8_t* st = p.stash + tile * kStashTileBytes + row * 16;
  uint8_t* tn = p.tan + tile * kTanTileBytes + row * 16;

  float e[4] = {0.f, 0.f, 0.f, 0.f}, off[3] = {0.f, 0.f, 0.f};
  float r = 0.f, w = 0.f;
  if (valid) {
#pragma unroll
    for (int d = 0; d < 3; ++d) { e[d] = p.e[pt * 3 + d]; off[d] = p.unmasked[pt * 3 + d]; }
    r = p.rigidity[pt];
    w = p.w[pt];
    if (p.w_is_alpha) w = 1.0f - expf(-fmaxf(w, 0.f));
  }
  {
    float hi[3], lo[3];
#pragma unroll
    for (int d = 0; d < 3; ++d) { hi[d] = __half2float(__float2half_rn(e[d])); lo[d] = e[d] - hi[d]; }
    *reinterpret_cast<uint4*>(tn + kTE) = make_uint4(pk(hi[0], hi[1]), pk(hi[2], lo[0]), pk(lo[1], lo[2]), 0u);
    const uint4 zz = make_uint4(0u, 0u, 0u, 0u);
#pragma unroll
    for (int c = 1; c < 6; ++c) *reinterpret_cast<uint4*>(tn + kTE + c * kChunkBytes) = zz;
  }
  const unsigned long long m1 = read_mask(st + kStHb1, 8), e1 = read_mask(st + kStHb1 + 8 * kChunkBytes, 4);
  const unsigned long long m2 = read_mask(st + kStHb2, 8), e2 = read_mask(st + kStHb2 + 8 * kChunkBytes, 4);
  const unsigned long long m3 = read_mask(st + kStHb3, 8), m4 = read_mask(st + kStHb4, 8);

  float t[64], s[32];
  matvec<4>(sw + kW0x, e, act, 64);
  take<64>(act, m1, 1.0f, t, tn + kT1);
  matvec<4>(sw + kR0, e, act, 32);
  take<32>(act, e1, 1.0f, s, tn + kT1 + 8 * kChunkBytes);
  matvec<64>(sw + kW1, t, act, 64);
  take<64>(act, m2, 1.0f, t, tn + kT2);
  matvec<32>(sw + kR1, s, act, 32);
  take<32>(act, e2, 1.0f, s, tn + kT2 + 8 * kChunkBytes);
  matvec<64>(sw + kW2, t, act, 64);
  take<64>(act, m3, 1.0f, t, tn + kT3);
  matvec<64>(sw + kW3, t, act, 64);
  take<64>(act, m4, 1.0f, t, tn + kT4);
  float tau_off[3] = {0.f, 0.f, 0.f}, tau_c = 0.f;
#pragma unroll
  for (int k = 0; k < 64; ++k) {
    tau_off[0] += sw[kW4 + k] * t[k]; tau_off[1] += sw[kW4 + 64 + k] * t[k]; tau_off[2] += sw[kW4 + 128 + k] * t[k];
  }
#pragma unroll
  for (int k = 0; k < 32; ++k) tau_c += sw[kR2 + k] * s[k];
  const float alpha = e[0] * tau_off[0] + e[1] * tau_off[1] + e[2] * tau_off[2];
  const float beta = e[0] * off[0] + e[1] * off[1] + e[2] * off[2];
  const float tau_r = 2.0f * r * (1.0f - r) * tau_c;
  const float d = r * alpha + beta * tau_r;
  if (valid) {
    p.d[pt] = d; p.adot[pt] = alpha; p.beta[pt] = beta; p.tauc[pt] = tau_c;
    atomicAdd(p.loss + pt / p.S, w * d * d / static_cast<float>(p.S));
  }
}

__global__ void __launch_bounds__(kDivThreads) div_bwd_kernel(const DivParams p) {
  extern __shared__ __align__(16) float sm[];
  float* sw = sm;
  float* act = sm + kWTotal + threadIdx.x;
  load_weights(sw, p);
  __syncthreads();
  const long long tile = blockIdx.x;
  const int row = threadIdx.x;
  const long long pt = tile * kTileM + row;
  const bool valid = pt < p.P;
  const uint8_t* st = p.stash + tile * kStashTileBytes + row * 16;
  uint8_t* ad = p.adj + tile * kAdjTileBytes + row * 16;

  float scale = 1.0f;
  {
    const float amax = p.amax ? __ldg(p.amax) : 0.f;
    if (amax > 0.f && amax < 3.0e38f) {
      int ex;
      frexpf(amax, &ex);
      scale = ldexpf(1.0f, min(max(10 - ex, -60), 60));
    }
  }
  float e[3] = {0.f, 0.f, 0.f};
  float r = 0.f, G = 0.f, alpha = 0.f, beta = 0.f, tau_c = 0.f;
  if (valid) {
#pragma unroll
    for (int d = 0; d < 3; ++d) e[d] = p.e[pt * 3 + d];
    r = p.rigidity[pt]; G = p.G[pt]; alpha = p.adot[pt]; beta = p.beta[pt]; tau_c = p.tauc[pt];
    const float rp = 2.0f * r * (1.0f - r);
    const float tau_r = rp * tau_c;
#pragma unroll
    for (int d = 0; d < 3; ++d) p.d_unmasked[pt * 3 + d] = G * tau_r * e[d];
    p.d_rigid[pt] = G * (alpha + 2.0f * beta * tau_c * (1.0f - 2.0f * r));
  }
  const float Gs = G * scale;
  const float rp = 2.0f * r * (1.0f - r);
  float tb_off[4] = {Gs * r * e[0], Gs * r * e[1], Gs * r * e[2], 0.f};
  const float tb_c = Gs * beta * rp;
  const uint4 zz = make_uint4(0u, 0u, 0u, 0u);
  *reinterpret_cast<uint4*>(ad + kA4) = make_uint4(pk(tb_off[0], tb_off[1]), pk(tb_off[2], 0.f), 0u, 0u);
  *reinterpret_cast<uint4*>(ad + kA4 + kChunkBytes) = zz;

  const unsigned long long m1 = read_mask(st + kStHb1, 8), e1 = read_mask(st + kStHb1 + 8 * kChunkBytes, 4);
  const unsigned long long m2 = read_mask(st + kStHb2, 8), e2 = read_mask(st + kStHb2 + 8 * kChunkBytes, 4);
  const unsigned long long m3 = read_mask(st + kStHb3, 8), m4 = read_mask(st + kStHb4, 8);

  float a[64], q[32];
#pragma unroll 1
  for (int k = 0; k < 64; ++k)
    act[k * kDivThreads] = sw[kW4 + k] * tb_off[0] + sw[kW4 + 64 + k] * tb_off[1] + sw[kW4 + 128 + k] * tb_off[2];
  take<64>(act, m4, 1.0f, a, ad + kA3);
  matvec_t<64>(sw + kW3, a, act, 64);
  take<64>(act, m3, 1.0f, a, ad + kA2);
  *reinterpret_cast<uint4*>(ad + kA2 + 8 * kChunkBytes) = make_uint4(pk(tb_c, 0.f), 0u, 0u, 0u);
  *reinterpret_cast<uint4*>(ad + kA2 + 9 * kChunkBytes) = zz;
  matvec_t<64>(sw + kW2, a, act, 64);
  take<64>(act, m2, 1.0f, a, ad + kA1);
#pragma unroll 1
  for (int k = 0; k < 32; ++k) act[k * kDivThreads] = sw[kR2 + k] * tb_c;
  take<32>(act, e2, 1.0f, q, ad + kA1 + 8 * kChunkBytes);
  matvec_t<64>(sw + kW1, a, act, 64);
  take<64>(act, m1, 1.0f, a, ad + kA0);
  matvec_t<32>(sw + kR1, q, act, 32);
  take<32>(act, e1, 1.0f, q, ad + kA0 + 8 * kChunkBytes);
}

static size_t div_smem() { return sizeof(float) * (kWTotal + kActFloats); }

namespace {
__global__ void div_G_kernel(const DivParams p, const float* __restrict__ g_ray, float* __restrict__ G, float* __restrict__ amax) {
  const long long pt = blockIdx.x * static_cast<long long>(blockDim.x) + threadIdx.x;
  float v = 0.f;
  if (pt < p.P) {
    float w = p.w[pt];
    if (p.w_is_alpha) w = 1.0f - expf(-fmaxf(w, 0.f));
    v = g_ray[pt / p.S] * (2.0f / static_cast<float>(p.S)) * w * p.d[pt];
    G[pt] = v;
  }
  float m = fabsf(v);
  if (!(m < 3.0e38f)) m = 0.f;
#pragma unroll
  for (int o = 16; o > 0; o >>= 1) m = fmaxf(m, __shfl_xor_sync(0xffffffffu, m, o));
  if ((threadIdx.x & 31) == 0 && m > 0.f) atomicMax(reinterpret_cast<int*>(amax), __float_as_int(m));
}
}

cudaError_t launch_div_G(const DivParams& p, const float* g_ray, float* G, float* amax, cudaStream_t st) {
  cudaError_t e = cudaMemsetAsync(amax, 0, sizeof(float), st);
  if (e != cudaSuccess || p.P <= 0) return e;
  div_G_kernel<<<static_cast<unsigned>((p.P + 255) / 256), 256, 0, st>>>(p, g_ray, G, amax);
  return cudaGetLastError();
}

cudaError_t launch_div_fwd(const DivParams& p, cudaStream_t st) {
  const long long tiles = (p.P + kTileM - 1) / kTileM;
  if (tiles <= 0) return cudaSuccess;
  cudaError_t e = cudaFuncSetAttribute(div_fwd_kernel, cudaFuncAttributeMaxDynamicSharedMemorySize, (int)div_smem());
  if (e != cudaSuccess) return e;
  div_fwd_kernel<<<static_cast<unsigned>(tiles), kDivThreads, div_smem(), st>>>(p);
  return cudaGetLastError();
}
cudaError_t launch_div_bwd(const DivParams& p, cudaStream_t st) {
  const long long tiles = (p.P + kTileM - 1) / kTileM;
  if (tiles <= 0) return cudaSuccess;
  cudaError_t e = cudaFuncSetAttribute(div_bwd_kernel, cudaFuncAttributeMaxDynamicSharedMemorySize, (int)div_smem());
  if (e != cudaSuccess) return e;
  div_bwd_kernel<<<static_cast<unsigned>(tiles), kDivThreads, div_smem(), st>>>(p);
  return cudaGetLastError();
}

}
```

nonrigid_nerf_b200/csrc/div.cuh:

```cuda
#pragma once
#include <cuda_runtime.h>
#include <stdint.h>

namespace nrn {

struct DivParams {
  long long P;
  int S, n_rays;
  const uint8_t* stash;
  const float* e;
  const float* unmasked;
  const float* rigidity;
  const float* w;
  int w_is_alpha;
  const float* net_w[5];
  const float* rig_w[3];
  uint8_t* tan;
  float* d;
  float* adot;
  float* beta;
  float* tauc;
  float* loss;
  const float* G;
  const float* amax;
  uint8_t* adj;
  float* d_unmasked;
  float* d_rigid;
};

cudaError_t launch_div_fwd(const DivParams& p, cudaStream_t st);
cudaError_t launch_div_bwd(const DivParams& p, cudaStream_t st);
cudaError_t launch_div_G(const DivParams& p, const float* g_ray, float* G, float* amax, cudaStream_t st);

}
```

nonrigid_nerf_b200/csrc/nrn_common.cuh:

```cuda
#pragma once
#include <cuda_runtime.h>
#include <stdint.h>

namespace nrn {

constexpr int kTileM = 128;
constexpr int kChunkBytes = kTileM * 16;
constexpr int kHBytes = 32 * kChunkBytes;
constexpr int kEBytes = 8 * kChunkBytes;
constexpr int kSlotBytes = kHBytes + kEBytes;
constexpr int kRingStageBytes = 32768;
constexpr int kRingStages = 4;
constexpr int kFwdThreads = 384;
constexpr int kProducerRegs = 40, kConsumerRegs = 232;

constexpr int kNerfL0Bytes = 8 * 256 * 16;
constexpr int kNerfLBytes = 32 * 256 * 16;
constexpr int kNerfL5Bytes = 40 * 256 * 16;
constexpr int kNerfHeadBytes = 32 * 16 * 16;
constexpr int kNerfWBytes = kNerfL0Bytes + 6 * kNerfLBytes + kNerfL5Bytes + kNerfHeadBytes;
constexpr int kNerfBiasFloats = 8 * 256 + 16;
constexpr int kNerfTOffset = kNerfWBytes + kNerfBiasFloats * 4;

constexpr int kBendB0Bytes = 6 * 96 * 16;
constexpr int kBendB1Bytes = 12 * 96 * 16;
constexpr int kBendB2Bytes = 12 * 80 * 16;
constexpr int kBendB3Bytes = 8 * 64 * 16;
constexpr int kBendB4Bytes = 8 * 16 * 16;
constexpr int kBendWBytes = kBendB0Bytes + kBendB1Bytes + kBendB2Bytes + kBendB3Bytes + kBendB4Bytes;
constexpr int kBendBiasFloats = 96 + 96 + 80 + 64;
constexpr int kBendTOffset = kBendWBytes + kBendBiasFloats * 4;
constexpr int kLatent = 32;

constexpr int kStE = 0;
constexpr int kStH = kStE + kEBytes;
constexpr int kStBin = kStH + 8 * kHBytes;
constexpr int kStHb1 = kStBin + 6 * kChunkBytes;
constexpr int kStHb2 = kStHb1 + 12 * kChunkBytes;
constexpr int kStHb3 = kStHb2 + 12 * kChunkBytes;
constexpr int kStHb4 = kStHb3 + 8 * kChunkBytes;
constexpr int kStashTileBytes = kStHb4 + 8 * kChunkBytes;

constexpr int kGsRaw = 0;
constexpr int kGsY = kGsRaw + 2 * kChunkBytes;
constexpr int kGsYb4 = kGsY + 8 * kHBytes;
constexpr int kGsYb3 = kGsYb4 + 2 * kChunkBytes;
constexpr int kGsYb2 = kGsYb3 + 8 * kChunkBytes;
constexpr int kGsYb1 = kGsYb2 + 10 * kChunkBytes;
constexpr int kGsYb0 = kGsYb1 + 12 * kChunkBytes;
constexpr int kGradTileBytes = kGsYb0 + 12 * kChunkBytes;
constexpr int kMaskHBytes = kTileM * 32;
constexpr int kMaskBBytes = kTileM * 16;
constexpr int kMkH = 0;
constexpr int kMkHb1 = kMkH + 8 * kMaskHBytes;
constexpr int kMkHb2 = kMkHb1 + kMaskBBytes;
constexpr int kMkHb3 = kMkHb2 + kMaskBBytes;
constexpr int kMkHb4 = kMkHb3 + kMaskBBytes;
constexpr int kMaskTileBytes = kMkHb4 + kMaskBBytes;
constexpr int kTanTileBytes = kStashTileBytes - kStBin;
constexpr int kAdjTileBytes = kGradTileBytes - kGsYb4;

constexpr int kNerfTHeadBytes = 2 * 256 * 16;
constexpr int kNerfTEBytes = 32 * 64 * 16;
constexpr int kNerfTWBytes = kNerfTHeadBytes + 7 * kNerfLBytes + 2 * kNerfTEBytes;
constexpr int kBendTB4Bytes = 2 * 64 * 16;
constexpr int kBendTB3Bytes = 8 * 64 * 16;
constexpr int kBendTB2Bytes = 10 * 96 * 16;
constexpr int kBendTB1Bytes = 12 * 96 * 16;
constexpr int kBendTB0Bytes = 12 * 48 * 16;
constexpr int kBendTWBytes = kBendTB4Bytes + kBendTB3Bytes + kBendTB2Bytes + kBendTB1Bytes + kBendTB0Bytes;
constexpr int kNerfPackedBytes = kNerfTOffset + kNerfTWBytes;
constexpr int kBendPackedBytes = kBendTOffset + kBendTWBytes;

struct FieldBwdParams {
  long long P;
  int n_tiles, S, n_rays, out_ch;
  const float* d_raw;
  const float* amax;
  const uint8_t* stash;
  uint8_t* gstash;
  const uint8_t* nerf_wT;
  const uint8_t* bend_wT;
  const float* unmasked;
  const float* rigidity;
  const float* d_unmasked_up;
  const float* d_rigid_up;
  float cutoff, scaling;
  int use_cutoff, use_scaling;
  float* d_latents;
  int* err;
  const uint8_t* relu_mask;
};

struct FieldFwdParams {
  const float* rays;
  const float* z_vals;
  const float* pts;
  long long pts_stride;
  const float* latents;
  long long latent_stride;
  int n_rays, S;
  long long P;
  int n_tiles;
  const uint8_t* nerf_w;
  const float* nerf_bias;
  const uint8_t* bend_w;
  const float* bend_bias;
  float cutoff, scaling, removal;
  int use_cutoff, use_scaling, use_removal;
  int out_ch;
  float* raw;
  float* d_init;
  float* d_bent;
  float* d_unmasked;
  float* d_masked;
  float* d_rigid;
  uint8_t* stash;
  int* err;
  uint8_t* relu_mask;
};

}
```

nonrigid_nerf_b200/csrc/pack.cu:

```cuda
#include <cuda_fp16.h>
#include "nrn_common.cuh"
#include "pack.cuh"

namespace nrn {

namespace {

__device__ __forceinline__ void decode(int idx, int R, int& k, int& r) {
  const int c = idx / (R * 8);
  const int rem = idx - c * R * 8;
  r = rem >> 3;
  k = c * 8 + (rem & 7);
}

__device__ __forceinline__ void pack_nerf_elem(const int idx, const NerfSrc& src, int in_ch, int out_ch, __half* __restrict__ w, float* __restrict__ bias) {
  constexpr int n0 = kNerfL0Bytes / 2, nl = kNerfLBytes / 2, n5 = kNerfL5Bytes / 2, nh = kNerfHeadBytes / 2;
  if (idx < kNerfWBytes / 2) {
    int i = idx, k, r;
    float v = 0.f;
    if (i < n0) {
      decode(i, 256, k, r);
      v = k < in_ch ? src.w[0][r * in_ch + k] : 0.f;
    } else if ((i -= n0) < 4 * nl) {
      const int L = 1 + i / nl;
      decode(i % nl, 256, k, r);
      v = src.w[L][r * 256 + k];
    } else if ((i -= 4 * nl) < n5) {
      decode(i, 256, k, r);
      const int ld = in_ch + 256;
      if (k < 64) v = k < in_ch ? src.w[5][r * ld + k] : 0.f;
      else v = src.w[5][r * ld + in_ch + (k - 64)];
    } else if ((i -= n5) < 2 * nl) {
      const int L = 6 + i / nl;
      decode(i % nl, 256, k, r);
      v = src.w[L][r * 256 + k];
    } else {
      i -= 2 * nl;
      decode(i, 16, k, r);
      v = r < out_ch ? src.w[8][r * 256 + k] : 0.f;
    }
    w[idx] = __float2half_rn(v);
  }
  if (idx < kNerfBiasFloats) {
    float b;
    if (idx < 2048) b = src.b[idx >> 8][idx & 255];
    else b = (idx - 2048) < out_ch ? src.b[8][idx - 2048] : 0.f;
    bias[idx] = b;
  }
  (void)nh;
}

__device__ __forceinline__ void pack_bender_elem(const int idx, const BenderSrc& src, __half* __restrict__ w, float* __restrict__ bias) {
  constexpr int n0 = kBendB0Bytes / 2, n1 = kBendB1Bytes / 2, n2 = kBendB2Bytes / 2, n3 = kBendB3Bytes / 2;
  constexpr int ld0 = 3 + kLatent;
  if (idx < kBendWBytes / 2) {
    int i = idx, k, r;
    float v = 0.f;
    if (i < n0) {
      decode(i, 96, k, r);
      if (r < 64) {
        if (k < 3) v = src.net_w[0][r * ld0 + k];
        else if (k < 6) v = src.net_w[0][r * ld0 + (k - 3)];
        else if (k < 6 + kLatent) v = src.net_w[0][r * ld0 + 3 + (k - 6)];
      } else {
        if (k < 3) v = src.rig_w[0][(r - 64) * 3 + k];
        else if (k < 6) v = src.rig_w[0][(r - 64) * 3 + (k - 3)];
      }
    } else if ((i -= n0) < n1) {
      decode(i, 96, k, r);
      if (r < 64) { if (k < 64) v = src.net_w[1][r * 64 + k]; }
      else { if (k >= 64) v = src.rig_w[1][(r - 64) * 32 + (k - 64)]; }
    } else if ((i -= n1) < n2) {
      decode(i, 80, k, r);
      if (r < 64) { if (k < 64) v = src.net_w[2][r * 64 + k]; }
      else if (r == 64) { if (k >= 64) v = src.rig_w[2][k - 64]; }
    } else if ((i -= n2) < n3) {
      decode(i, 64, k, r);
      v = src.net_w[3][r * 64 + k];
    } else {
      i -= n3;
      decode(i, 16, k, r);
      if (r < 3) v = src.net_w[4][r * 64 + k];
    }
    w[idx] = __float2half_rn(v);
  }
  if (idx < kBendBiasFloats) {
    float b = 0.f;
    if (idx < 96) b = idx < 64 ? src.net_b[0][idx] : src.rig_b[0][idx - 64];
    else if (idx < 192) { const int j = idx - 96; b = j < 64 ? src.net_b[1][j] : src.rig_b[1][j - 64]; }
    else if (idx < 272) { const int j = idx - 192; b = j < 64 ? src.net_b[2][j] : (j == 64 ? src.rig_b[2][0] : 0.f); }
    else b = src.net_b[3][idx - 272];
    bias[idx] = b;
  }
}

__device__ __forceinline__ void pack_nerf_t_elem(const int idx, const NerfSrc& src, int in_ch, int out_ch, __half* __restrict__ w) {
  if (idx >= kNerfTWBytes / 2) return;
  constexpr int nh = kNerfTHeadBytes / 2, nl = kNerfLBytes / 2, ne = kNerfTEBytes / 2;
  int i = idx, k, r;
  float v = 0.f;
  const int ld5 = in_ch + 256;
  if (i < nh) {
    decode(i, 256, k, r);
    v = k < out_ch ? src.w[8][k * 256 + r] : 0.f;
  } else if ((i -= nh) < 2 * nl) {
    const int L = 7 - i / nl;
    decode(i % nl, 256, k, r);
    v = src.w[L][k * 256 + r];
  } else if ((i -= 2 * nl) < ne) {
    decode(i, 64, k, r);
    v = r < in_ch ? src.w[5][k * ld5 + r] : 0.f;
  } else if ((i -= ne) < nl) {
    decode(i, 256, k, r);
    v = src.w[5][k * ld5 + in_ch + r];
  } else if ((i -= nl) < 4 * nl) {
    const int L = 4 - i / nl;
    decode(i % nl, 256, k, r);
    v = src.w[L][k * 256 + r];
  } else {
    i -= 4 * nl;
    decode(i, 64, k, r);
    v = r < in_ch ? src.w[0][k * in_ch + r] : 0.f;
  }
  w[idx] = __float2half_rn(v);
}

__device__ __forceinline__ void pack_bender_t_elem(const int idx, const BenderSrc& src, __half* __restrict__ w) {
  if (idx >= kBendTWBytes / 2) return;
  constexpr int n4 = kBendTB4Bytes / 2, n3 = kBendTB3Bytes / 2, n2 = kBendTB2Bytes / 2, n1 = kBendTB1Bytes / 2;
  constexpr int ld0 = 3 + kLatent;
  int i = idx, k, r;
  float v = 0.f;
  if (i < n4) {
    decode(i, 64, k, r);
    v = k < 3 ? src.net_w[4][k * 64 + r] : 0.f;
  } else if ((i -= n4) < n3) {
    decode(i, 64, k, r);
    v = src.net_w[3][k * 64 + r];
  } else if ((i -= n3) < n2) {
    decode(i, 96, k, r);
    if (r < 64) { if (k < 64) v = src.net_w[2][k * 64 + r]; }
    else { if (k == 64) v = src.rig_w[2][r - 64]; }
  } else if ((i -= n2) < n1) {
    decode(i, 96, k, r);
    if (r < 64) { if (k < 64) v = src.net_w[1][k * 64 + r]; }
    else { if (k >= 64) v = src.rig_w[1][(k - 64) * 32 + (r - 64)]; }
  } else {
    i -= n1;
    decode(i, 48, k, r);
    if (r >= 6 && r < 6 + kLatent) { if (k < 64) v = src.net_w[0][k * ld0 + 3 + (r - 6)]; }
    else if (r < 3) v = k < 64 ? src.net_w[0][k * ld0 + r] : src.rig_w[0][(k - 64) * 3 + r];
  }
  w[idx] = __float2half_rn(v);
}


constexpr int kPackThreads = 256;
__global__ void __launch_bounds__(kPackThreads) pack_nerf_kernel(NerfSrc src, int in_ch, int out_ch, __half* __restrict__ w,
                                                                 float* __restrict__ bias, __half* __restrict__ wt) {
  constexpr int nb_fwd = (kNerfWBytes / 2 + kPackThreads - 1) / kPackThreads;
  if (blockIdx.x < nb_fwd) pack_nerf_elem(blockIdx.x * kPackThreads + threadIdx.x, src, in_ch, out_ch, w, bias);
  else pack_nerf_t_elem((blockIdx.x - nb_fwd) * kPackThreads + threadIdx.x, src, in_ch, out_ch, wt);
}
__global__ void __launch_bounds__(kPackThreads) pack_bender_kernel(BenderSrc src, __half* __restrict__ w, float* __restrict__ bias,
                                                                   __half* __restrict__ wt) {
  constexpr int nb_fwd = (kBendWBytes / 2 + kPackThreads - 1) / kPackThreads;
  if (blockIdx.x < nb_fwd) pack_bender_elem(blockIdx.x * kPackThreads + threadIdx.x, src, w, bias);
  else pack_bender_t_elem((blockIdx.x - nb_fwd) * kPackThreads + threadIdx.x, src, wt);
}

}

cudaError_t launch_pack_nerf(const NerfSrc& src, int in_ch, int out_ch, void* packed, cudaStream_t st) {
  uint8_t* base = reinterpret_cast<uint8_t*>(packed);
  const int nb = (kNerfWBytes / 2 + kPackThreads - 1) / kPackThreads + (kNerfTWBytes / 2 + kPackThreads - 1) / kPackThreads;
  pack_nerf_kernel<<<nb, kPackThreads, 0, st>>>(src, in_ch, out_ch, reinterpret_cast<__half*>(base),
                                               reinterpret_cast<float*>(base + kNerfWBytes), reinterpret_cast<__half*>(base + kNerfTOffset));
  return cudaGetLastError();
}
cudaError_t launch_pack_bender(const BenderSrc& src, void* packed, cudaStream_t st) {
  uint8_t* base = reinterpret_cast<uint8_t*>(packed);
  const int nb = (kBendWBytes / 2 + kPackThreads - 1) / kPackThreads + (kBendTWBytes / 2 + kPackThreads - 1) / kPackThreads;
  pack_bender_kernel<<<nb, kPackThreads, 0, st>>>(src, reinterpret_cast<__half*>(base), reinterpret_cast<float*>(base + kBendWBytes),
                                                 reinterpret_cast<__half*>(base + kBendTOffset));
  return cudaGetLastError();
}

}
```

Measured before the change: 369,900.

## Move divergence kernels to split-fp16 wgmma with TMA-resident packed bender weights

Rewrites the divergence forward and backward kernels to run the bender MLP tangent/adjoint passes on wgmma tensor cores instead of scalar fp32 matvecs. To keep close to fp32 accuracy, weights and activations are split into hi/lo fp16 halves, with the lo part scaled. The packed bender layout gains lo-weight sections, and the kernels load them into shared memory via TMA bulk copies. The kernels now read compact ReLU masks instead of the full activation stash and run as a persistent grid sized to the SM count. This adds packing work and ABI changes, and numerics now depend on the split-precision scheme.

```diff
diff --git a/include/nrnerf_b200.h b/include/nrnerf_b200.h
--- a/include/nrnerf_b200.h
+++ b/include/nrnerf_b200.h
@@ -8,7 +8,7 @@
 extern "C" {
 #endif
 
-#define NRN_ABI_VERSION 3
+#define NRN_ABI_VERSION 4
 
 #define NRN_OK 0
 #define NRN_E_INVALID (-1)
@@ -132,14 +132,13 @@
 size_t nrn_div_grad_stash_bytes(int n_rays, int n_samples);
 typedef struct NrnDivArgs {
   int32_t n_rays, n_samples;
-  const void* stash;
+  const void* relu_mask;
   const float* e;
   const float* unmasked_offsets;
   const float* rigidity_mask;
   const float* weights;
   int32_t weights_are_opacity_alpha;
-  const float* const* net_w;
-  const float* const* rig_w;
+  const void* bender_packed;
   void* tangent_stash;
   float* d; float* alpha; float* beta; float* tau_c;
   float* loss;
diff --git a/nonrigid_nerf_b200/_lib.py b/nonrigid_nerf_b200/_lib.py
--- a/nonrigid_nerf_b200/_lib.py
+++ b/nonrigid_nerf_b200/_lib.py
@@ -6,7 +6,7 @@
 
 _HERE = os.path.dirname(os.path.abspath(__file__))
 LIB_PATH = os.path.join(_HERE, "libnrnerf_b200.so")
-ABI_VERSION = 3
+ABI_VERSION = 4
 
 _f32p = C.POINTER(C.c_float)
 _vp = C.c_void_p
@@ -48,9 +48,9 @@
 class NrnDivArgs(C.Structure):
     _fields_ = [
         ("n_rays", C.c_int32), ("n_samples", C.c_int32),
-        ("stash", _vp), ("e", _vp), ("unmasked_offsets", _vp), ("rigidity_mask", _vp), ("weights", _vp),
+        ("relu_mask", _vp), ("e", _vp), ("unmasked_offsets", _vp), ("rigidity_mask", _vp), ("weights", _vp),
         ("weights_are_opacity_alpha", C.c_int32),
-        ("net_w", C.POINTER(_vp)), ("rig_w", C.POINTER(_vp)),
+        ("bender_packed", _vp),
         ("tangent_stash", _vp), ("d", _vp), ("alpha", _vp), ("beta", _vp), ("tau_c", _vp), ("loss", _vp),
         ("G", _vp), ("g_ray", _vp), ("G_workspace", _vp), ("adjoint_stash", _vp), ("wgrad_scratch", _vp), ("d_unmasked_offsets", _vp),
         ("d_rigidity_mask", _vp), ("bender_grad", _vp),
diff --git a/nonrigid_nerf_b200/autograd.py b/nonrigid_nerf_b200/autograd.py
--- a/nonrigid_nerf_b200/autograd.py
+++ b/nonrigid_nerf_b200/autograd.py
@@ -69,7 +69,7 @@
         ctx.params = params
         ctx.set_materialize_grads(False)
         if bender is not None:
-            _register_stash(det["unmasked_offsets"], stash)
+            _register_relu_mask(det["unmasked_offsets"], relu_mask)
             ctx.save_for_backward(det["unmasked_offsets"], det["rigidity_mask"])
             outs = (raw, det["unmasked_offsets"], det["rigidity_mask"], det["initial_input_pts"], det["input_pts"],
                     det["masked_offsets"])
@@ -203,34 +203,34 @@
     return _LatentGatherFn.apply(timestep, *latents)
 
 
-_STASH_BY_PTR = {}
-
-
-def _register_stash(unmasked: torch.Tensor, stash: torch.Tensor) -> None:
+_MASK_BY_PTR = {}
+
+
+def _register_relu_mask(unmasked: torch.Tensor, relu_mask: torch.Tensor) -> None:
     import weakref
-    for k in [k for k, v in _STASH_BY_PTR.items() if v() is None]:
-        del _STASH_BY_PTR[k]
-    _STASH_BY_PTR[unmasked.data_ptr()] = weakref.ref(stash)
-
-
-def lookup_stash(unmasked: torch.Tensor) -> Optional[torch.Tensor]:
+    for k in [k for k, v in _MASK_BY_PTR.items() if v() is None]:
+        del _MASK_BY_PTR[k]
+    _MASK_BY_PTR[unmasked.data_ptr()] = weakref.ref(relu_mask)
+
+
+def lookup_relu_mask(unmasked: torch.Tensor) -> Optional[torch.Tensor]:
     fn = unmasked.grad_fn
     for _ in range(8):
         if fn is None:
             break
-        stash = getattr(fn, "stash", None)
-        if isinstance(stash, torch.Tensor):
-            return stash
+        relu_mask = getattr(fn, "relu_mask", None)
+        if isinstance(relu_mask, torch.Tensor):
+            return relu_mask
         nxt = [f for f, _ in fn.next_functions if f is not None]
         fn = nxt[0] if len(nxt) == 1 else None
-    ref = _STASH_BY_PTR.get(unmasked.data_ptr())
+    ref = _MASK_BY_PTR.get(unmasked.data_ptr())
     return ref() if ref is not None else None
 
 
 class _DivergenceFn(torch.autograd.Function):
 
     @staticmethod
-    def forward(ctx, unmasked, rigidity, weights, e, stash, bender, w_is_alpha, *bend_p):
+    def forward(ctx, unmasked, rigidity, weights, e, relu_mask, bender, w_is_alpha, *bend_p):
         n, s = unmasked.shape[0], unmasked.shape[1]
         dev = unmasked.device
         lib = _lib.load()
@@ -240,22 +240,20 @@
         rg = rigidity.detach().contiguous().float()
         w = weights.detach().contiguous().float()
         e = e.contiguous().float()
-        net_w, _, rig_w, _ = ops.bender_param_list(bender)
-        net_arr = ops._ptr_array([t.detach() for t in net_w])
-        rig_arr = ops._ptr_array([t.detach() for t in rig_w])
+        bender_pack = ops.pack_bender(bender)
         tan = torch.empty(lib.nrn_div_stash_bytes(n, s), dtype=torch.uint8, device=dev)
         scal = torch.empty(4, n * s, dtype=torch.float32, device=dev)
         loss = torch.empty(n, dtype=torch.float32, device=dev)
-        a.stash, a.e, a.unmasked_offsets, a.rigidity_mask, a.weights = stash.data_ptr(), e.data_ptr(), un.data_ptr(), rg.data_ptr(), w.data_ptr()
+        a.relu_mask, a.e, a.unmasked_offsets, a.rigidity_mask, a.weights = relu_mask.data_ptr(), e.data_ptr(), un.data_ptr(), rg.data_ptr(), w.data_ptr()
         a.weights_are_opacity_alpha = 1 if w_is_alpha else 0
-        a.net_w, a.rig_w = net_arr, rig_arr
+        a.bender_packed = bender_pack.data_ptr()
         a.tangent_stash = tan.data_ptr()
         a.d, a.alpha, a.beta, a.tau_c = (scal[i].data_ptr() for i in range(4))
         a.loss = loss.data_ptr()
         a.stream = torch.cuda.current_stream().cuda_stream
         with torch.cuda.device(dev):
             _lib.check(lib.nrn_divergence_forward(C.byref(a)), "divergence_forward")
-        ctx.keep = (un, rg, w, e, stash, tan, scal, bender)
+        ctx.keep = (un, rg, w, e, relu_mask, bender_pack, tan, scal, bender)
         ctx.bend_p = bend_p
         ctx.w_is_alpha = bool(w_is_alpha)
         ctx.shape = (n, s)
@@ -264,7 +262,7 @@
 
     @staticmethod
     def backward(ctx, g):
-        un, rg, w, e, stash, tan, scal, bender = ctx.keep
+        un, rg, w, e, relu_mask, bender_pack, tan, scal, bender = ctx.keep
         n, s = ctx.shape
         dev = un.device
         lib = _lib.load()
@@ -272,12 +270,9 @@
         G = torch.empty(n * s, dtype=torch.float32, device=dev)
         a = _lib.NrnDivArgs()
         a.n_rays, a.n_samples = n, s
-        net_w, _, rig_w, _ = ops.bender_param_list(bender)
-        net_arr = ops._ptr_array([t.detach() for t in net_w])
-        rig_arr = ops._ptr_array([t.detach() for t in rig_w])
-        a.stash, a.e, a.unmasked_offsets, a.rigidity_mask, a.weights = stash.data_ptr(), e.data_ptr(), un.data_ptr(), rg.data_ptr(), w.data_ptr()
+        a.relu_mask, a.e, a.unmasked_offsets, a.rigidity_mask, a.weights = relu_mask.data_ptr(), e.data_ptr(), un.data_ptr(), rg.data_ptr(), w.data_ptr()
         a.weights_are_opacity_alpha = 1 if ctx.w_is_alpha else 0
-        a.net_w, a.rig_w = net_arr, rig_arr
+        a.bender_packed = bender_pack.data_ptr()
         a.tangent_stash = tan.data_ptr()
         a.d, a.alpha, a.beta, a.tau_c = (scal[i].data_ptr() for i in range(4))
         a.g_ray, a.G_workspace = g.data_ptr(), G.data_ptr()
@@ -307,17 +302,17 @@
 
 def divergence_loss(unmasked: torch.Tensor, rigidity: torch.Tensor, weights: Optional[torch.Tensor], bender,
                     e: Optional[torch.Tensor] = None, opacity_alpha: Optional[torch.Tensor] = None) -> torch.Tensor:
-    stash = lookup_stash(unmasked)
-    if stash is None:
-        raise RuntimeError("nonrigid_nerf_b200: no activation stash for these offsets -- the fused divergence term needs the "
+    relu_mask = lookup_relu_mask(unmasked)
+    if relu_mask is None:
+        raise RuntimeError("nonrigid_nerf_b200: no ReLU masks for these offsets -- the fused divergence term needs the "
                            "un-chunked coarse pass of the current differentiable render() call (N_rand <= chunk)")
     n, s = unmasked.shape[0], unmasked.shape[1]
     if e is None:
         e = torch.randn(n * s, 3, device=unmasked.device)
     _, bend_p = _flat_params_bender(bender)
     if opacity_alpha is not None:
-        return _DivergenceFn.apply(unmasked, rigidity, opacity_alpha, e, stash, bender, True, *bend_p)
-    return _DivergenceFn.apply(unmasked, rigidity, weights, e, stash, bender, False, *bend_p)
+        return _DivergenceFn.apply(unmasked, rigidity, opacity_alpha, e, relu_mask, bender, True, *bend_p)
+    return _DivergenceFn.apply(unmasked, rigidity, weights, e, relu_mask, bender, False, *bend_p)
 
 
 def _flat_params_bender(bender):
diff --git a/nonrigid_nerf_b200/csrc/c_abi.cu b/nonrigid_nerf_b200/csrc/c_abi.cu
--- a/nonrigid_nerf_b200/csrc/c_abi.cu
+++ b/nonrigid_nerf_b200/csrc/c_abi.cu
@@ -358,15 +358,17 @@
 static int fill_div(const NrnDivArgs* a, nrn::DivParams& p, const char* who) {
   if (!a) return fail(NRN_E_INVALID, "%s: null args", who);
   if (a->n_rays < 0 || a->n_samples < 1) return fail(NRN_E_INVALID, "%s: bad sizes", who);
-  if (!a->stash || !a->e || !a->unmasked_offsets || !a->rigidity_mask || !a->weights || !a->net_w || !a->rig_w || !a->tangent_stash ||
-      !a->d || !a->alpha || !a->beta || !a->tau_c)
+  if (!a->relu_mask) return fail(NRN_E_INVALID, "%s: null relu_mask (the ReLU masks of the coarse nrn_field_forward call)", who);
+  if (!a->bender_packed) return fail(NRN_E_INVALID, "%s: null bender_packed (the nrn_pack_bender output the coarse pass ran with)", who);
+  if (!aligned16(a->bender_packed)) return fail(NRN_E_INVALID, "%s: bender_packed must be 16-byte aligned", who);
+  if (!a->e || !a->unmasked_offsets || !a->rigidity_mask || !a->weights || !a->tangent_stash || !a->d || !a->alpha || !a->beta ||
+      !a->tau_c)
     return fail(NRN_E_INVALID, "%s: null argument", who);
   p.P = static_cast<long long>(a->n_rays) * a->n_samples;
   p.S = a->n_samples; p.n_rays = a->n_rays;
-  p.stash = static_cast<const uint8_t*>(a->stash);
+  p.relu_mask = static_cast<const uint8_t*>(a->relu_mask);
+  p.bender = static_cast<const uint8_t*>(a->bender_packed);
   p.e = a->e; p.unmasked = a->unmasked_offsets; p.rigidity = a->rigidity_mask; p.w = a->weights; p.w_is_alpha = a->weights_are_opacity_alpha != 0;
-  for (int i = 0; i < 5; ++i) { if (!a->net_w[i]) return fail(NRN_E_INVALID, "%s: null weight", who); p.net_w[i] = a->net_w[i]; }
-  for (int i = 0; i < 3; ++i) { if (!a->rig_w[i]) return fail(NRN_E_INVALID, "%s: null weight", who); p.rig_w[i] = a->rig_w[i]; }
   p.tan = static_cast<uint8_t*>(a->tangent_stash);
   p.d = a->d; p.adot = a->alpha; p.beta = a->beta; p.tauc = a->tau_c;
   return NRN_OK;
@@ -377,11 +379,15 @@
   int rc = fill_div(a, p, "nrn_divergence_forward");
   if (rc) return rc;
   if (!a->loss) return fail(NRN_E_INVALID, "nrn_divergence_forward: null loss");
+  DeviceState* ds;
+  rc = device_state(&ds);
+  if (rc) return rc;
+  p.err = ds->err_word;
   cudaStream_t st = static_cast<cudaStream_t>(a->stream);
   cudaError_t e = cudaMemsetAsync(a->loss, 0, sizeof(float) * static_cast<size_t>(a->n_rays), st);
   if (e != cudaSuccess) return cuda_fail(e, "memset loss");
   p.loss = a->loss;
-  { ScopedTimer tm(5, st); e = nrn::launch_div_fwd(p, st); }
+  { ScopedTimer tm(5, st); e = nrn::launch_div_fwd(p, ds->num_sms, st); }
   return e == cudaSuccess ? NRN_OK : cuda_fail(e, "div_fwd_kernel");
 }
 
@@ -398,10 +404,10 @@
   cudaStream_t st = static_cast<cudaStream_t>(a->stream);
   float* amax = reinterpret_cast<float*>(ds->err_word + 2);
   p.G = a->G ? a->G : a->G_workspace; p.amax = amax; p.adj = static_cast<uint8_t*>(a->adjoint_stash);
-  p.d_unmasked = a->d_unmasked_offsets; p.d_rigid = a->d_rigidity_mask;
+  p.d_unmasked = a->d_unmasked_offsets; p.d_rigid = a->d_rigidity_mask; p.err = ds->err_word;
   cudaError_t e = a->G ? nrn::launch_absmax(a->G, p.P, amax, st) : nrn::launch_div_G(p, a->g_ray, a->G_workspace, amax, st);
   if (e != cudaSuccess) return cuda_fail(e, "absmax_kernel");
-  { ScopedTimer tm(5, st); e = nrn::launch_div_bwd(p, st); }
+  { ScopedTimer tm(5, st); e = nrn::launch_div_bwd(p, ds->num_sms, st); }
   if (e != cudaSuccess) return cuda_fail(e, "div_bwd_kernel");
   nrn::WgradParams w{};
   w.stash = p.tan; w.gstash = p.adj; w.scratch = a->wgrad_scratch; w.amax = amax; w.compact = 1;
diff --git a/nonrigid_nerf_b200/csrc/div.cu b/nonrigid_nerf_b200/csrc/div.cu
--- a/nonrigid_nerf_b200/csrc/div.cu
+++ b/nonrigid_nerf_b200/csrc/div.cu
@@ -1,183 +1,261 @@
-#include <cuda_fp16.h>
-#include "nrn_common.cuh"
+#include "field_mma.cuh"
 #include "div.cuh"
 
 namespace nrn {
 
 namespace {
 
-constexpr int kDivThreads = 128;
-constexpr int kW0x = 0;
-constexpr int kW1 = kW0x + 64 * 4;
-constexpr int kW2 = kW1 + 4096;
-constexpr int kW3 = kW2 + 4096;
-constexpr int kW4 = kW3 + 4096;
-constexpr int kR0 = kW4 + 192;
-constexpr int kR1 = kR0 + 128;
-constexpr int kR2 = kR1 + 1024;
-constexpr int kWTotal = kR2 + 32;
-constexpr int kActFloats = 64 * kDivThreads;
+constexpr int kDivTilesPerCta = 2;
+constexpr int kDivWgs = 2 * kDivTilesPerCta;
+constexpr int kDivThreads = 128 * kDivWgs;
+constexpr int kDivStageLd = 12;
+constexpr int kDivImgBytes = 12 * kChunkBytes;
+constexpr float kLoInv = 1.0f / kBendLoScale;
 
 constexpr int kTE = 0, kT1 = 6 * kChunkBytes, kT2 = 18 * kChunkBytes, kT3 = 30 * kChunkBytes, kT4 = 38 * kChunkBytes;
 constexpr int kA4 = 0, kA3 = 2 * kChunkBytes, kA2 = 10 * kChunkBytes, kA1 = 20 * kChunkBytes, kA0 = 32 * kChunkBytes;
 
-__device__ __forceinline__ void load_weights(float* sw, const DivParams& p) {
-  for (int i = threadIdx.x; i < 64 * 4; i += blockDim.x) sw[kW0x + i] = (i & 3) < 3 ? p.net_w[0][(i >> 2) * 35 + (i & 3)] : 0.f;
-  for (int i = threadIdx.x; i < 4096; i += blockDim.x) {
-    sw[kW1 + i] = p.net_w[1][i];
-    sw[kW2 + i] = p.net_w[2][i];
-    sw[kW3 + i] = p.net_w[3][i];
-  }
-  for (int i = threadIdx.x; i < 192; i += blockDim.x) sw[kW4 + i] = p.net_w[4][i];
-  for (int i = threadIdx.x; i < 32 * 4; i += blockDim.x) sw[kR0 + i] = (i & 3) < 3 ? p.rig_w[0][(i >> 2) * 3 + (i & 3)] : 0.f;
-  for (int i = threadIdx.x; i < 1024; i += blockDim.x) sw[kR1 + i] = p.rig_w[1][i];
-  for (int i = threadIdx.x; i < 32; i += blockDim.x) sw[kR2 + i] = p.rig_w[2][i];
-}
-
-__device__ __forceinline__ unsigned long long read_mask(const uint8_t* row, int nchunks) {
-  unsigned long long m = 0ull;
-  for (int c = 0; c < nchunks; ++c) {
-    const uint4 w = __ldg(reinterpret_cast<const uint4*>(row + c * kChunkBytes));
-    const uint32_t ww[4] = {w.x, w.y, w.z, w.w};
-#pragma unroll
-    for (int q = 0; q < 4; ++q) {
-      if (ww[q] & 0x7fffu) m |= 1ull << (c * 8 + 2 * q);
-      if (ww[q] & 0x7fff0000u) m |= 1ull << (c * 8 + 2 * q + 1);
-    }
-  }
-  return m;
-}
-
-__device__ __forceinline__ uint32_t pk(float a, float b) {
-  __half2 h = __floats2half2_rn(fminf(fmaxf(a, -65504.f), 65504.f), fminf(fmaxf(b, -65504.f), 65504.f));
-  return *reinterpret_cast<uint32_t*>(&h);
-}
-
-template <int IN>
-__device__ __forceinline__ void matvec(const float* W, const float (&in)[IN], float* act, int OUT) {
+constexpr int kDivFwdWBytes = kBendWBytes;
+constexpr int kDivBwdWBytes = kBendTB4Bytes + kBendTB3Bytes + kBendTB2Bytes + kBendTB1Bytes;
+
+struct DivShared {
+  uint64_t w_full;
+  int abort_flag;
+};
+
+constexpr size_t div_smem_bytes(int wbytes) {
+  return 2 * kDivTilesPerCta * kDivImgBytes + 2 * wbytes + kDivWgs * kWgRows * kDivStageLd * sizeof(float) + sizeof(DivShared);
+}
+static_assert(div_smem_bytes(kDivFwdWBytes) <= 227 * 1024, "div kernels: shared memory of one CTA per SM");
+
+struct DivSmem {
+  uint8_t* img_hi;
+  uint8_t* img_lo;
+  uint8_t* w_hi;
+  uint8_t* w_lo;
+  float* stage;
+  DivShared* sh;
+};
+__device__ __forceinline__ DivSmem div_smem(uint8_t* smem, int wbytes, int wg) {
+  DivSmem s;
+  s.img_hi = smem + (wg >> 1) * 2 * kDivImgBytes;
+  s.img_lo = s.img_hi + kDivImgBytes;
+  s.w_hi = smem + 2 * kDivTilesPerCta * kDivImgBytes;
+  s.w_lo = s.w_hi + wbytes;
+  float* stage_all = reinterpret_cast<float*>(s.w_lo + wbytes);
+  s.stage = stage_all + wg * kWgRows * kDivStageLd;
+  s.sh = reinterpret_cast<DivShared*>(stage_all + kDivWgs * kWgRows * kDivStageLd);
+  return s;
+}
+
+__device__ __forceinline__ void load_resident_weights(const DivSmem& s, const uint8_t* hi, const uint8_t* lo, uint32_t bytes) {
+  if (threadIdx.x == 0) {
+    mbar_init(&s.sh->w_full, 1);
+    s.sh->abort_flag = 0;
+    fence_mbar_init();
+  }
+  __syncthreads();
+  if (threadIdx.x == 0) {
+    mbar_arrive_expect_tx(&s.sh->w_full, 2 * bytes);
+    for (uint32_t off = 0; off < bytes; off += 16384u) {
+      tma_bulk_g2s(s.w_hi + off, hi + off, min(bytes - off, 16384u), &s.sh->w_full);
+      tma_bulk_g2s(s.w_lo + off, lo + off, min(bytes - off, 16384u), &s.sh->w_full);
+    }
+  }
+}
+
+template <int N, bool A_LO>
+__device__ __forceinline__ void wg_mma_split(float (&acc)[N / 2], uint32_t a_hi, uint32_t a_lo, const DivSmem& s, uint32_t w_off,
+                                             uint32_t k16) {
+  const uint64_t ahi = gmma_desc(a_hi, kChunkBytes, 128), alo = gmma_desc(a_lo, kChunkBytes, 128);
+  const uint64_t whi = gmma_desc(smem_u32(s.w_hi) + w_off, N * 16, 128), wlo = gmma_desc(smem_u32(s.w_lo) + w_off, N * 16, 128);
+#pragma unroll
+  for (int i = 0; i < N / 2; ++i) acc[i] = 0.f;
+  acc_fence(acc);
+  wgmma_fence();
 #pragma unroll 1
-  for (int j0 = 0; j0 < OUT; j0 += 4) {
-    float a0 = 0.f, a1 = 0.f, a2 = 0.f, a3 = 0.f;
-#pragma unroll
-    for (int k = 0; k < IN; k += 4) {
-      const float4 w0 = *reinterpret_cast<const float4*>(W + (j0 + 0) * IN + k);
-      const float4 w1 = *reinterpret_cast<const float4*>(W + (j0 + 1) * IN + k);
-      const float4 w2 = *reinterpret_cast<const float4*>(W + (j0 + 2) * IN + k);
-      const float4 w3 = *reinterpret_cast<const float4*>(W + (j0 + 3) * IN + k);
-      a0 += w0.x * in[k] + w0.y * in[k + 1] + w0.z * in[k + 2] + w0.w * in[k + 3];
-      a1 += w1.x * in[k] + w1.y * in[k + 1] + w1.z * in[k + 2] + w1.w * in[k + 3];
-      a2 += w2.x * in[k] + w2.y * in[k + 1] + w2.z * in[k + 2] + w2.w * in[k + 3];
-      a3 += w3.x * in[k] + w3.y * in[k + 1] + w3.z * in[k + 2] + w3.w * in[k + 3];
-    }
-    act[(j0 + 0) * kDivThreads] = a0; act[(j0 + 1) * kDivThreads] = a1;
-    act[(j0 + 2) * kDivThreads] = a2; act[(j0 + 3) * kDivThreads] = a3;
-  }
-}
-template <int NJ>
-__device__ __forceinline__ void matvec_t(const float* W, const float (&in)[NJ], float* act, int NK) {
+  for (uint32_t k = 0; k < k16; ++k) {
+    if (A_LO) wgmma<N, 0, 0>(acc, gmma_desc_advance(alo, k * 2 * kChunkBytes), gmma_desc_advance(whi, k * 2 * N * 16), 1u);
+    wgmma<N, 0, 0>(acc, gmma_desc_advance(ahi, k * 2 * kChunkBytes), gmma_desc_advance(wlo, k * 2 * N * 16), 1u);
+  }
+  wgmma_commit();
+  wgmma_wait<0>();
+  acc_fence(acc);
+#pragma unroll
+  for (int i = 0; i < N / 2; ++i) acc[i] *= kLoInv;
+  acc_fence(acc);
+  wgmma_fence();
 #pragma unroll 1
-  for (int k0 = 0; k0 < NK; k0 += 4) {
-    float a0 = 0.f, a1 = 0.f, a2 = 0.f, a3 = 0.f;
-#pragma unroll
-    for (int j = 0; j < NJ; ++j) {
-      const float4 w = *reinterpret_cast<const float4*>(W + j * NK + k0);
-      a0 += w.x * in[j]; a1 += w.y * in[j]; a2 += w.z * in[j]; a3 += w.w * in[j];
-    }
-    act[(k0 + 0) * kDivThreads] = a0; act[(k0 + 1) * kDivThreads] = a1;
-    act[(k0 + 2) * kDivThreads] = a2; act[(k0 + 3) * kDivThreads] = a3;
-  }
-}
-template <int N>
-__device__ __forceinline__ void take(const float* act, unsigned long long mask, float scale, float (&out)[N], uint8_t* img_row) {
-#pragma unroll
-  for (int j = 0; j < N; ++j) out[j] = ((mask >> j) & 1ull) ? act[j * kDivThreads] * scale : 0.f;
-#pragma unroll
-  for (int c = 0; c < N / 8; ++c) {
-    const uint4 v = make_uint4(pk(out[c * 8], out[c * 8 + 1]), pk(out[c * 8 + 2], out[c * 8 + 3]), pk(out[c * 8 + 4], out[c * 8 + 5]),
-                               pk(out[c * 8 + 6], out[c * 8 + 7]));
-    *reinterpret_cast<uint4*>(img_row + c * kChunkBytes) = v;
-  }
-}
-
-}
-
-__global__ void __launch_bounds__(kDivThreads) div_fwd_kernel(const DivParams p) {
-  extern __shared__ __align__(16) float sm[];
-  float* sw = sm;
-  float* act = sm + kWTotal + threadIdx.x;
-  load_weights(sw, p);
-  __syncthreads();
-  const long long tile = blockIdx.x;
-  const int row = threadIdx.x;
-  const long long pt = tile * kTileM + row;
-  const bool valid = pt < p.P;
-  const uint8_t* st = p.stash + tile * kStashTileBytes + row * 16;
-  uint8_t* tn = p.tan + tile * kTanTileBytes + row * 16;
-
-  float e[4] = {0.f, 0.f, 0.f, 0.f}, off[3] = {0.f, 0.f, 0.f};
-  float r = 0.f, w = 0.f;
-  if (valid) {
-#pragma unroll
-    for (int d = 0; d < 3; ++d) { e[d] = p.e[pt * 3 + d]; off[d] = p.unmasked[pt * 3 + d]; }
-    r = p.rigidity[pt];
-    w = p.w[pt];
-    if (p.w_is_alpha) w = 1.0f - expf(-fmaxf(w, 0.f));
-  }
-  {
-    float hi[3], lo[3];
-#pragma unroll
-    for (int d = 0; d < 3; ++d) { hi[d] = __half2float(__float2half_rn(e[d])); lo[d] = e[d] - hi[d]; }
-    *reinterpret_cast<uint4*>(tn + kTE) = make_uint4(pk(hi[0], hi[1]), pk(hi[2], lo[0]), pk(lo[1], lo[2]), 0u);
-    const uint4 zz = make_uint4(0u, 0u, 0u, 0u);
-#pragma unroll
-    for (int c = 1; c < 6; ++c) *reinterpret_cast<uint4*>(tn + kTE + c * kChunkBytes) = zz;
-  }
-  const unsigned long long m1 = read_mask(st + kStHb1, 8), e1 = read_mask(st + kStHb1 + 8 * kChunkBytes, 4);
-  const unsigned long long m2 = read_mask(st + kStHb2, 8), e2 = read_mask(st + kStHb2 + 8 * kChunkBytes, 4);
-  const unsigned long long m3 = read_mask(st + kStHb3, 8), m4 = read_mask(st + kStHb4, 8);
-
-  float t[64], s[32];
-  matvec<4>(sw + kW0x, e, act, 64);
-  take<64>(act, m1, 1.0f, t, tn + kT1);
-  matvec<4>(sw + kR0, e, act, 32);
-  take<32>(act, e1, 1.0f, s, tn + kT1 + 8 * kChunkBytes);
-  matvec<64>(sw + kW1, t, act, 64);
-  take<64>(act, m2, 1.0f, t, tn + kT2);
-  matvec<32>(sw + kR1, s, act, 32);
-  take<32>(act, e2, 1.0f, s, tn + kT2 + 8 * kChunkBytes);
-  matvec<64>(sw + kW2, t, act, 64);
-  take<64>(act, m3, 1.0f, t, tn + kT3);
-  matvec<64>(sw + kW3, t, act, 64);
-  take<64>(act, m4, 1.0f, t, tn + kT4);
-  float tau_off[3] = {0.f, 0.f, 0.f}, tau_c = 0.f;
-#pragma unroll
-  for (int k = 0; k < 64; ++k) {
-    tau_off[0] += sw[kW4 + k] * t[k]; tau_off[1] += sw[kW4 + 64 + k] * t[k]; tau_off[2] += sw[kW4 + 128 + k] * t[k];
-  }
-#pragma unroll
-  for (int k = 0; k < 32; ++k) tau_c += sw[kR2 + k] * s[k];
-  const float alpha = e[0] * tau_off[0] + e[1] * tau_off[1] + e[2] * tau_off[2];
-  const float beta = e[0] * off[0] + e[1] * off[1] + e[2] * off[2];
-  const float tau_r = 2.0f * r * (1.0f - r) * tau_c;
-  const float d = r * alpha + beta * tau_r;
-  if (valid) {
-    p.d[pt] = d; p.adot[pt] = alpha; p.beta[pt] = beta; p.tauc[pt] = tau_c;
-    atomicAdd(p.loss + pt / p.S, w * d * d / static_cast<float>(p.S));
-  }
-}
-
-__global__ void __launch_bounds__(kDivThreads) div_bwd_kernel(const DivParams p) {
-  extern __shared__ __align__(16) float sm[];
-  float* sw = sm;
-  float* act = sm + kWTotal + threadIdx.x;
-  load_weights(sw, p);
-  __syncthreads();
-  const long long tile = blockIdx.x;
-  const int row = threadIdx.x;
-  const long long pt = tile * kTileM + row;
-  const bool valid = pt < p.P;
-  const uint8_t* st = p.stash + tile * kStashTileBytes + row * 16;
-  uint8_t* ad = p.adj + tile * kAdjTileBytes + row * 16;
+  for (uint32_t k = 0; k < k16; ++k)
+    wgmma<N, 0, 0>(acc, gmma_desc_advance(ahi, k * 2 * kChunkBytes), gmma_desc_advance(whi, k * 2 * N * 16), 1u);
+  wgmma_commit();
+  wgmma_wait<0>();
+  acc_fence(acc);
+}
+
+__device__ __forceinline__ uint2 split_h2(float a, float b) {
+  const uint32_t hi = pack_h2_sat(a, b);
+  const float2 h = __half22float2(*reinterpret_cast<const __half2*>(&hi));
+  return make_uint2(hi, pack_h2_sat((a - h.x) * kBendLoScale, (b - h.y) * kBendLoScale));
+}
+
+template <int NCOLS, int NR>
+__device__ __forceinline__ void epi_mask_split(const float (&acc)[NR], const ReluMask<NCOLS>& m, const DivSmem& s, int h) {
+  const int r0 = h * kWgRows + acc_r0(), q = acc_q();
+#pragma unroll
+  for (int j = 0; j < NCOLS / 8; ++j) {
+#pragma unroll
+    for (int i = 0; i < 2; ++i) {
+      const uint2 v = split_h2(acc[4 * j + 2 * i], acc[4 * j + 2 * i + 1]);
+      const int off = j * kChunkBytes + (r0 + 8 * i) * 16 + 4 * q;
+      *reinterpret_cast<uint32_t*>(s.img_hi + off) = m.apply(i, j, v.x);
+      *reinterpret_cast<uint32_t*>(s.img_lo + off) = m.apply(i, j, v.y);
+    }
+  }
+}
+
+}
+
+__global__ void __launch_bounds__(kDivThreads, 1) div_fwd_kernel(const DivParams p) {
+  extern __shared__ __align__(128) uint8_t smem[];
+  const int wg = threadIdx.x >> 7;
+  const int h = wg & 1;
+  const DivSmem s = div_smem(smem, kDivFwdWBytes, wg);
+  load_resident_weights(s, p.bender, p.bender + kBendLoOffset, kDivFwdWBytes);
+  const Waiter W{&s.sh->abort_flag, p.err};
+
+  const int tw = threadIdx.x & 127;
+  const int lane = threadIdx.x & 31;
+  const bool row_thread = tw < kWgRows;
+  const int bar = 1 + wg;
+  const bool wg_leader = tw == 0;
+  const int row_off = (h * kWgRows + tw) * 16;
+  const uint32_t a_hi = smem_u32(s.img_hi) + h * kWgRows * 16, a_lo = smem_u32(s.img_lo) + h * kWgRows * 16;
+  constexpr uint32_t w_b0 = 0, w_b1 = w_b0 + kBendB0Bytes, w_b2 = w_b1 + kBendB1Bytes, w_b3 = w_b2 + kBendB2Bytes,
+                     w_b4 = w_b3 + kBendB3Bytes;
+  const float* my_stg = s.stage + tw * kDivStageLd;
+  const long long n_tiles = (p.P + kTileM - 1) / kTileM;
+
+  for (long long tile = static_cast<long long>(blockIdx.x) * kDivTilesPerCta + (wg >> 1); tile < n_tiles;
+       tile += static_cast<long long>(gridDim.x) * kDivTilesPerCta) {
+    const long long pt = tile * kTileM + h * kWgRows + tw;
+    const bool valid = row_thread && pt < p.P;
+    uint8_t* tn = p.tan + tile * kTanTileBytes;
+    const uint8_t* mk = p.relu_mask + tile * kMaskTileBytes;
+    auto stash_begin = [&]() {
+      if (wg_leader) tma_bulk_wait_read<0>();
+      wg_bar(bar);
+    };
+    auto ready = [&](uint32_t off, uint32_t chunks) {
+      fence_proxy_async_smem();
+      wg_bar(bar);
+      if (wg_leader) store_rows(tn + off, s.img_hi, h, chunks);
+    };
+
+    float e[3] = {0.f, 0.f, 0.f}, off[3] = {0.f, 0.f, 0.f};
+    float r = 0.f, w = 0.f;
+    if (valid) {
+#pragma unroll
+      for (int d = 0; d < 3; ++d) { e[d] = __ldg(p.e + pt * 3 + d); off[d] = __ldg(p.unmasked + pt * 3 + d); }
+      r = __ldg(p.rigidity + pt);
+      w = __ldg(p.w + pt);
+      if (p.w_is_alpha) w = 1.0f - expf(-fmaxf(w, 0.f));
+    }
+    stash_begin();
+    if (row_thread) {
+      float hi[3], lo[3];
+#pragma unroll
+      for (int d = 0; d < 3; ++d) { hi[d] = __half2float(__float2half_rn(e[d])); lo[d] = e[d] - hi[d]; }
+      uint8_t* a_row = s.img_hi + row_off;
+      *reinterpret_cast<uint4*>(a_row) = make_uint4(pack_h2(hi[0], hi[1]), pack_h2(hi[2], lo[0]), pack_h2(lo[1], lo[2]), 0u);
+#pragma unroll
+      for (int c = 1; c < 6; ++c) *reinterpret_cast<uint4*>(a_row + c * kChunkBytes) = make_uint4(0u, 0u, 0u, 0u);
+    }
+    ready(kTE, 6);
+    {
+      float acc[48];
+      ReluMask<96> m;
+      m.load(mk + kMkHb1, h);
+      W.wait(&s.sh->w_full, 0, 330);
+      wg_mma_split<96, false>(acc, a_hi, a_lo, s, w_b0, 3);
+      stash_begin();
+      epi_mask_split<96>(acc, m, s, h);
+      ready(kT1, 12);
+      m.load(mk + kMkHb2, h);
+      wg_mma_split<96, true>(acc, a_hi, a_lo, s, w_b1, 6);
+      stash_begin();
+      epi_mask_split<96>(acc, m, s, h);
+      ready(kT2, 12);
+    }
+    {
+      float acc[40];
+      ReluMask<64> m;
+      m.load(mk + kMkHb3, h);
+      wg_mma_split<80, true>(acc, a_hi, a_lo, s, w_b2, 6);
+      stash_begin();
+      epi_mask_split<64>(acc, m, s, h);
+      if (acc_q() == 0) {
+        s.stage[acc_r0() * kDivStageLd + 8] = acc[32];
+        s.stage[(acc_r0() + 8) * kDivStageLd + 8] = acc[34];
+      }
+      ready(kT3, 8);
+    }
+    {
+      float acc[32];
+      ReluMask<64> m;
+      m.load(mk + kMkHb4, h);
+      wg_mma_split<64, true>(acc, a_hi, a_lo, s, w_b3, 4);
+      stash_begin();
+      epi_mask_split<64>(acc, m, s, h);
+      ready(kT4, 8);
+    }
+    {
+      float acc[8];
+      wg_mma_split<16, true>(acc, a_hi, a_lo, s, w_b4, 4);
+      stage_cols<0, 1>(acc, s.stage, kDivStageLd);
+      wg_bar(bar);
+      if (row_thread) {
+        const float tau_c = my_stg[8];
+        const float alpha = e[0] * my_stg[0] + e[1] * my_stg[1] + e[2] * my_stg[2];
+        const float beta = e[0] * off[0] + e[1] * off[1] + e[2] * off[2];
+        const float tau_r = 2.0f * r * (1.0f - r) * tau_c;
+        const float d = r * alpha + beta * tau_r;
+        float part = 0.f;
+        if (valid) {
+          p.d[pt] = d; p.adot[pt] = alpha; p.beta[pt] = beta; p.tauc[pt] = tau_c;
+          part = w * d * d / static_cast<float>(p.S);
+        }
+        const long long ray = valid ? pt / p.S : -1;
+        const long long ray0 = __shfl_sync(0xffffffffu, ray, 0);
+        if (__all_sync(0xffffffffu, valid && ray == ray0)) {
+#pragma unroll
+          for (int o = 16; o > 0; o >>= 1) part += __shfl_xor_sync(0xffffffffu, part, o);
+          if (lane == 0) atomicAdd(p.loss + ray0, part);
+        } else if (valid) {
+          atomicAdd(p.loss + ray, part);
+        }
+      }
+    }
+  }
+  if (wg_leader) tma_bulk_wait<0>();
+}
+
+__global__ void __launch_bounds__(kDivThreads, 1) div_bwd_kernel(const DivParams p) {
+  extern __shared__ __align__(128) uint8_t smem[];
+  const int wg = threadIdx.x >> 7;
+  const int h = wg & 1;
+  const DivSmem s = div_smem(smem, kDivBwdWBytes, wg);
+  load_resident_weights(s, p.bender + kBendTOffset, p.bender + kBendTLoOffset, kDivBwdWBytes);
+  const Waiter W{&s.sh->abort_flag, p.err};
+
+  const int tw = threadIdx.x & 127;
+  const bool row_thread = tw < kWgRows;
+  const int bar = 1 + wg;
+  const bool wg_leader = tw == 0;
+  const int row_off = (h * kWgRows + tw) * 16;
+  const uint32_t a_hi = smem_u32(s.img_hi) + h * kWgRows * 16, a_lo = smem_u32(s.img_lo) + h * kWgRows * 16;
+  constexpr uint32_t w_t4 = 0, w_t3 = w_t4 + kBendTB4Bytes, w_t2 = w_t3 + kBendTB3Bytes, w_t1 = w_t2 + kBendTB2Bytes;
+  const long long n_tiles = (p.P + kTileM - 1) / kTileM;
 
   float scale = 1.0f;
   {
@@ -188,51 +266,86 @@
       scale = ldexpf(1.0f, min(max(10 - ex, -60), 60));
     }
   }
-  float e[3] = {0.f, 0.f, 0.f};
-  float r = 0.f, G = 0.f, alpha = 0.f, beta = 0.f, tau_c = 0.f;
-  if (valid) {
-#pragma unroll
-    for (int d = 0; d < 3; ++d) e[d] = p.e[pt * 3 + d];
-    r = p.rigidity[pt]; G = p.G[pt]; alpha = p.adot[pt]; beta = p.beta[pt]; tau_c = p.tauc[pt];
+
+  for (long long tile = static_cast<long long>(blockIdx.x) * kDivTilesPerCta + (wg >> 1); tile < n_tiles;
+       tile += static_cast<long long>(gridDim.x) * kDivTilesPerCta) {
+    const long long pt = tile * kTileM + h * kWgRows + tw;
+    const bool valid = row_thread && pt < p.P;
+    uint8_t* ad = p.adj + tile * kAdjTileBytes;
+    const uint8_t* mk = p.relu_mask + tile * kMaskTileBytes;
+    auto stash_begin = [&]() {
+      if (wg_leader) tma_bulk_wait_read<0>();
+      wg_bar(bar);
+    };
+    auto ready = [&](uint32_t off, uint32_t chunks) {
+      fence_proxy_async_smem();
+      wg_bar(bar);
+      if (wg_leader) store_rows(ad + off, s.img_hi, h, chunks);
+    };
+
+    float e[3] = {0.f, 0.f, 0.f};
+    float r = 0.f, G = 0.f, beta = 0.f;
+    if (valid) {
+#pragma unroll
+      for (int d = 0; d < 3; ++d) e[d] = __ldg(p.e + pt * 3 + d);
+      r = __ldg(p.rigidity + pt); G = __ldg(p.G + pt); beta = __ldg(p.beta + pt);
+      const float alpha = __ldg(p.adot + pt), tau_c = __ldg(p.tauc + pt);
+      const float tau_r = 2.0f * r * (1.0f - r) * tau_c;
+#pragma unroll
+      for (int d = 0; d < 3; ++d) p.d_unmasked[pt * 3 + d] = G * tau_r * e[d];
+      p.d_rigid[pt] = G * (alpha + 2.0f * beta * tau_c * (1.0f - 2.0f * r));
+    }
+    const float Gs = G * scale;
     const float rp = 2.0f * r * (1.0f - r);
-    const float tau_r = rp * tau_c;
-#pragma unroll
-    for (int d = 0; d < 3; ++d) p.d_unmasked[pt * 3 + d] = G * tau_r * e[d];
-    p.d_rigid[pt] = G * (alpha + 2.0f * beta * tau_c * (1.0f - 2.0f * r));
-  }
-  const float Gs = G * scale;
-  const float rp = 2.0f * r * (1.0f - r);
-  float tb_off[4] = {Gs * r * e[0], Gs * r * e[1], Gs * r * e[2], 0.f};
-  const float tb_c = Gs * beta * rp;
-  const uint4 zz = make_uint4(0u, 0u, 0u, 0u);
-  *reinterpret_cast<uint4*>(ad + kA4) = make_uint4(pk(tb_off[0], tb_off[1]), pk(tb_off[2], 0.f), 0u, 0u);
-  *reinterpret_cast<uint4*>(ad + kA4 + kChunkBytes) = zz;
-
-  const unsigned long long m1 = read_mask(st + kStHb1, 8), e1 = read_mask(st + kStHb1 + 8 * kChunkBytes, 4);
-  const unsigned long long m2 = read_mask(st + kStHb2, 8), e2 = read_mask(st + kStHb2 + 8 * kChunkBytes, 4);
-  const unsigned long long m3 = read_mask(st + kStHb3, 8), m4 = read_mask(st + kStHb4, 8);
-
-  float a[64], q[32];
-#pragma unroll 1
-  for (int k = 0; k < 64; ++k)
-    act[k * kDivThreads] = sw[kW4 + k] * tb_off[0] + sw[kW4 + 64 + k] * tb_off[1] + sw[kW4 + 128 + k] * tb_off[2];
-  take<64>(act, m4, 1.0f, a, ad + kA3);
-  matvec_t<64>(sw + kW3, a, act, 64);
-  take<64>(act, m3, 1.0f, a, ad + kA2);
-  *reinterpret_cast<uint4*>(ad + kA2 + 8 * kChunkBytes) = make_uint4(pk(tb_c, 0.f), 0u, 0u, 0u);
-  *reinterpret_cast<uint4*>(ad + kA2 + 9 * kChunkBytes) = zz;
-  matvec_t<64>(sw + kW2, a, act, 64);
-  take<64>(act, m2, 1.0f, a, ad + kA1);
-#pragma unroll 1
-  for (int k = 0; k < 32; ++k) act[k * kDivThreads] = sw[kR2 + k] * tb_c;
-  take<32>(act, e2, 1.0f, q, ad + kA1 + 8 * kChunkBytes);
-  matvec_t<64>(sw + kW1, a, act, 64);
-  take<64>(act, m1, 1.0f, a, ad + kA0);
-  matvec_t<32>(sw + kR1, q, act, 32);
-  take<32>(act, e1, 1.0f, q, ad + kA0 + 8 * kChunkBytes);
-}
-
-static size_t div_smem() { return sizeof(float) * (kWTotal + kActFloats); }
+    const float tb_c = Gs * beta * rp;
+    stash_begin();
+    if (row_thread) {
+      const uint2 t01 = split_h2(Gs * r * e[0], Gs * r * e[1]), t2 = split_h2(Gs * r * e[2], 0.f);
+      *reinterpret_cast<uint4*>(s.img_hi + row_off) = make_uint4(t01.x, t2.x, 0u, 0u);
+      *reinterpret_cast<uint4*>(s.img_lo + row_off) = make_uint4(t01.y, t2.y, 0u, 0u);
+      *reinterpret_cast<uint4*>(s.img_hi + row_off + kChunkBytes) = make_uint4(0u, 0u, 0u, 0u);
+      *reinterpret_cast<uint4*>(s.img_lo + row_off + kChunkBytes) = make_uint4(0u, 0u, 0u, 0u);
+    }
+    ready(kA4, 2);
+    {
+      float acc[32];
+      ReluMask<64> m;
+      m.load(mk + kMkHb4, h);
+      W.wait(&s.sh->w_full, 0, 340);
+      wg_mma_split<64, true>(acc, a_hi, a_lo, s, w_t4, 1);
+      stash_begin();
+      epi_mask_split<64>(acc, m, s, h);
+      ready(kA3, 8);
+      m.load(mk + kMkHb3, h);
+      wg_mma_split<64, true>(acc, a_hi, a_lo, s, w_t3, 4);
+      stash_begin();
+      epi_mask_split<64>(acc, m, s, h);
+      if (row_thread) {
+        const uint2 t = split_h2(tb_c, 0.f);
+        *reinterpret_cast<uint4*>(s.img_hi + row_off + 8 * kChunkBytes) = make_uint4(t.x, 0u, 0u, 0u);
+        *reinterpret_cast<uint4*>(s.img_lo + row_off + 8 * kChunkBytes) = make_uint4(t.y, 0u, 0u, 0u);
+        *reinterpret_cast<uint4*>(s.img_hi + row_off + 9 * kChunkBytes) = make_uint4(0u, 0u, 0u, 0u);
+        *reinterpret_cast<uint4*>(s.img_lo + row_off + 9 * kChunkBytes) = make_uint4(0u, 0u, 0u, 0u);
+      }
+      ready(kA2, 10);
+    }
+    {
+      float acc[48];
+      ReluMask<96> m;
+      m.load(mk + kMkHb2, h);
+      wg_mma_split<96, true>(acc, a_hi, a_lo, s, w_t2, 5);
+      stash_begin();
+      epi_mask_split<96>(acc, m, s, h);
+      ready(kA1, 12);
+      m.load(mk + kMkHb1, h);
+      wg_mma_split<96, true>(acc, a_hi, a_lo, s, w_t1, 6);
+      stash_begin();
+      epi_mask_split<96>(acc, m, s, h);
+      ready(kA0, 12);
+    }
+  }
+  if (wg_leader) tma_bulk_wait<0>();
+}
 
 namespace {
 __global__ void div_G_kernel(const DivParams p, const float* __restrict__ g_ray, float* __restrict__ G, float* __restrict__ amax) {
@@ -250,6 +363,18 @@
   for (int o = 16; o > 0; o >>= 1) m = fmaxf(m, __shfl_xor_sync(0xffffffffu, m, o));
   if ((threadIdx.x & 31) == 0 && m > 0.f) atomicMax(reinterpret_cast<int*>(amax), __float_as_int(m));
 }
+
+template <typename Kernel>
+cudaError_t launch_div(Kernel kernel, int wbytes, const DivParams& p, int num_sms, cudaStream_t st) {
+  const long long tiles = (p.P + kTileM - 1) / kTileM;
+  if (tiles <= 0) return cudaSuccess;
+  const int smem = static_cast<int>(div_smem_bytes(wbytes));
+  cudaError_t e = cudaFuncSetAttribute(kernel, cudaFuncAttributeMaxDynamicSharedMemorySize, smem);
+  if (e != cudaSuccess) return e;
+  const long long pairs = (tiles + kDivTilesPerCta - 1) / kDivTilesPerCta;
+  kernel<<<static_cast<unsigned>(pairs < num_sms ? pairs : num_sms), kDivThreads, smem, st>>>(p);
+  return cudaGetLastError();
+}
 }
 
 cudaError_t launch_div_G(const DivParams& p, const float* g_ray, float* G, float* amax, cudaStream_t st) {
@@ -259,21 +384,11 @@
   return cudaGetLastError();
 }
 
-cudaError_t launch_div_fwd(const DivParams& p, cudaStream_t st) {
-  const long long tiles = (p.P + kTileM - 1) / kTileM;
-  if (tiles <= 0) return cudaSuccess;
-  cudaError_t e = cudaFuncSetAttribute(div_fwd_kernel, cudaFuncAttributeMaxDynamicSharedMemorySize, (int)div_smem());
-  if (e != cudaSuccess) return e;
-  div_fwd_kernel<<<static_cast<unsigned>(tiles), kDivThreads, div_smem(), st>>>(p);
-  return cudaGetLastError();
-}
-cudaError_t launch_div_bwd(const DivParams& p, cudaStream_t st) {
-  const long long tiles = (p.P + kTileM - 1) / kTileM;
-  if (tiles <= 0) return cudaSuccess;
-  cudaError_t e = cudaFuncSetAttribute(div_bwd_kernel, cudaFuncAttributeMaxDynamicSharedMemorySize, (int)div_smem());
-  if (e != cudaSuccess) return e;
-  div_bwd_kernel<<<static_cast<unsigned>(tiles), kDivThreads, div_smem(), st>>>(p);
-  return cudaGetLastError();
-}
-
-}
+cudaError_t launch_div_fwd(const DivParams& p, int num_sms, cudaStream_t st) {
+  return launch_div(div_fwd_kernel, kDivFwdWBytes, p, num_sms, st);
+}
+cudaError_t launch_div_bwd(const DivParams& p, int num_sms, cudaStream_t st) {
+  return launch_div(div_bwd_kernel, kDivBwdWBytes, p, num_sms, st);
+}
+
+}
diff --git a/nonrigid_nerf_b200/csrc/div.cuh b/nonrigid_nerf_b200/csrc/div.cuh
--- a/nonrigid_nerf_b200/csrc/div.cuh
+++ b/nonrigid_nerf_b200/csrc/div.cuh
@@ -7,14 +7,13 @@
 struct DivParams {
   long long P;
   int S, n_rays;
-  const uint8_t* stash;
+  const uint8_t* relu_mask;
+  const uint8_t* bender;
   const float* e;
   const float* unmasked;
   const float* rigidity;
   const float* w;
   int w_is_alpha;
-  const float* net_w[5];
-  const float* rig_w[3];
   uint8_t* tan;
   float* d;
   float* adot;
@@ -26,10 +25,11 @@
   uint8_t* adj;
   float* d_unmasked;
   float* d_rigid;
+  int* err;
 };
 
-cudaError_t launch_div_fwd(const DivParams& p, cudaStream_t st);
-cudaError_t launch_div_bwd(const DivParams& p, cudaStream_t st);
+cudaError_t launch_div_fwd(const DivParams& p, int num_sms, cudaStream_t st);
+cudaError_t launch_div_bwd(const DivParams& p, int num_sms, cudaStream_t st);
 cudaError_t launch_div_G(const DivParams& p, const float* g_ray, float* G, float* amax, cudaStream_t st);
 
 }
diff --git a/nonrigid_nerf_b200/csrc/nrn_common.cuh b/nonrigid_nerf_b200/csrc/nrn_common.cuh
--- a/nonrigid_nerf_b200/csrc/nrn_common.cuh
+++ b/nonrigid_nerf_b200/csrc/nrn_common.cuh
@@ -70,7 +70,10 @@
 constexpr int kBendTB0Bytes = 12 * 48 * 16;
 constexpr int kBendTWBytes = kBendTB4Bytes + kBendTB3Bytes + kBendTB2Bytes + kBendTB1Bytes + kBendTB0Bytes;
 constexpr int kNerfPackedBytes = kNerfTOffset + kNerfTWBytes;
-constexpr int kBendPackedBytes = kBendTOffset + kBendTWBytes;
+constexpr float kBendLoScale = 2048.f;
+constexpr int kBendLoOffset = kBendTOffset + kBendTWBytes;
+constexpr int kBendTLoOffset = kBendLoOffset + kBendWBytes;
+constexpr int kBendPackedBytes = kBendTLoOffset + kBendTWBytes;
 
 struct FieldBwdParams {
   long long P;
diff --git a/nonrigid_nerf_b200/csrc/pack.cu b/nonrigid_nerf_b200/csrc/pack.cu
--- a/nonrigid_nerf_b200/csrc/pack.cu
+++ b/nonrigid_nerf_b200/csrc/pack.cu
@@ -50,7 +50,10 @@
   (void)nh;
 }
 
-__device__ __forceinline__ void pack_bender_elem(const int idx, const BenderSrc& src, __half* __restrict__ w, float* __restrict__ bias) {
+__device__ __forceinline__ __half lo_half(float v) { return __float2half_rn((v - __half2float(__float2half_rn(v))) * kBendLoScale); }
+
+__device__ __forceinline__ void pack_bender_elem(const int idx, const BenderSrc& src, __half* __restrict__ w, float* __restrict__ bias,
+                                                 __half* __restrict__ wlo) {
   constexpr int n0 = kBendB0Bytes / 2, n1 = kBendB1Bytes / 2, n2 = kBendB2Bytes / 2, n3 = kBendB3Bytes / 2;
   constexpr int ld0 = 3 + kLatent;
   if (idx < kBendWBytes / 2) {
@@ -83,6 +86,7 @@
       if (r < 3) v = src.net_w[4][r * 64 + k];
     }
     w[idx] = __float2half_rn(v);
+    wlo[idx] = lo_half(v);
   }
   if (idx < kBendBiasFloats) {
     float b = 0.f;
@@ -125,7 +129,7 @@
   w[idx] = __float2half_rn(v);
 }
 
-__device__ __forceinline__ void pack_bender_t_elem(const int idx, const BenderSrc& src, __half* __restrict__ w) {
+__device__ __forceinline__ void pack_bender_t_elem(const int idx, const BenderSrc& src, __half* __restrict__ w, __half* __restrict__ wlo) {
   if (idx >= kBendTWBytes / 2) return;
   constexpr int n4 = kBendTB4Bytes / 2, n3 = kBendTB3Bytes / 2, n2 = kBendTB2Bytes / 2, n1 = kBendTB1Bytes / 2;
   constexpr int ld0 = 3 + kLatent;
@@ -152,6 +156,7 @@
     else if (r < 3) v = k < 64 ? src.net_w[0][k * ld0 + r] : src.rig_w[0][(k - 64) * 3 + r];
   }
   w[idx] = __float2half_rn(v);
+  wlo[idx] = lo_half(v);
 }
 
 
@@ -163,10 +168,11 @@
   else pack_nerf_t_elem((blockIdx.x - nb_fwd) * kPackThreads + threadIdx.x, src, in_ch, out_ch, wt);
 }
 __global__ void __launch_bounds__(kPackThreads) pack_bender_kernel(BenderSrc src, __half* __restrict__ w, float* __restrict__ bias,
-                                                                   __half* __restrict__ wt) {
+                                                                   __half* __restrict__ wt, __half* __restrict__ wlo,
+                                                                   __half* __restrict__ wtlo) {
   constexpr int nb_fwd = (kBendWBytes / 2 + kPackThreads - 1) / kPackThreads;
-  if (blockIdx.x < nb_fwd) pack_bender_elem(blockIdx.x * kPackThreads + threadIdx.x, src, w, bias);
-  else pack_bender_t_elem((blockIdx.x - nb_fwd) * kPackThreads + threadIdx.x, src, wt);
+  if (blockIdx.x < nb_fwd) pack_bender_elem(blockIdx.x * kPackThreads + threadIdx.x, src, w, bias, wlo);
+  else pack_bender_t_elem((blockIdx.x - nb_fwd) * kPackThreads + threadIdx.x, src, wt, wtlo);
 }
 
 }
@@ -182,7 +188,8 @@
   uint8_t* base = reinterpret_cast<uint8_t*>(packed);
   const int nb = (kBendWBytes / 2 + kPackThreads - 1) / kPackThreads + (kBendTWBytes / 2 + kPackThreads - 1) / kPackThreads;
   pack_bender_kernel<<<nb, kPackThreads, 0, st>>>(src, reinterpret_cast<__half*>(base), reinterpret_cast<float*>(base + kBendWBytes),
-                                                 reinterpret_cast<__half*>(base + kBendTOffset));
+                                                 reinterpret_cast<__half*>(base + kBendTOffset), reinterpret_cast<__half*>(base + kBendLoOffset),
+                                                 reinterpret_cast<__half*>(base + kBendTLoOffset));
   return cudaGetLastError();
 }
 
```

Result: faster. 396,900, median of 6 (+7.3%).
